# B1ueber2y/DIST-Renderer

Hardware: NVIDIA B200
Metric: rays/sec (fwd+bwd) (higher is better)
Workload: dtype f32 (split-fp16 tensor-core operands, fp32 accumulate)

## Files before the change

### dist-renderer_b200/csrc/common.cuh

```cuda
#pragma once
#include <cuda_runtime.h>
#include <stdint.h>
#include "../../include/dist_b200.h"

namespace dist {

void set_error(const char* fmt, ...);
int num_sms();
void count_launch();

#define DIST_CHECK_CUDA(expr)                                                                   \
  do {                                                                                          \
    cudaError_t _e = (expr);                                                                    \
    if (_e != cudaSuccess) {                                                                    \
      ::dist::set_error("%s failed: %s (%s:%d)", #expr, cudaGetErrorString(_e), __FILE__, __LINE__); \
      return DIST_E_CUDA;                                                                       \
    }                                                                                           \
  } while (0)

#define DIST_REQUIRE(cond, ...)                 \
  do {                                          \
    if (!(cond)) {                              \
      ::dist::set_error(__VA_ARGS__);           \
      return DIST_E_INVALID;                    \
    }                                           \
  } while (0)

__host__ __device__ inline int round_up(int x, int m) { return (x + m - 1) / m * m; }

struct NetDev {
  int n_layers, latent_in, use_tanh;
  int K[DIST_MAX_LAYERS], N[DIST_MAX_LAYERS];
  const float* Wt[DIST_MAX_LAYERS];
  const float* W[DIST_MAX_LAYERS];
  const float* bias[DIST_MAX_LAYERS];
};

int make_netdev(const dist_net_t* net, NetDev* out);

struct MlpArgs {
  const float* points;
  int64_t n_host;
  const int32_t* n_dev;
  float clamp_dist;
  float* sdf;
  float* grad;
  const float* coef;
  const uint8_t* use_clamp;
  float* acc0;
  float* accl;
  int64_t* rows_evaluated;
  int64_t n2_host;
  const int32_t* n2_dev;
  int64_t seg2_offset;
  int screen_seg1;
  float screen_thresh;
  uint8_t* seg_approx;
  unsigned long long* tile_counters;
  uint32_t* mask_buf;
  int64_t mask_cap;
  int64_t mask_base_host;
  const int32_t* mask_base_dev;
  const int32_t* slots;
  const float* sdf_in;
};
int mlp_simt_launch(const NetDev& net, int mode, const MlpArgs& a, cudaStream_t stream);
int mlp_tc_launch(const dist_net_t* net, const NetDev& nd, int mode, const MlpArgs& a, cudaStream_t stream);

int mlp_launch(const dist_net_t* net, const NetDev& nd, int engine, int mode, const MlpArgs& a, cudaStream_t stream);

}
```

### dist-renderer_b200/csrc/march.cu

```cuda
#include <cuda_runtime.h>
#include <math.h>
#include <string.h>
#include "common.cuh"

namespace dist {
namespace {

struct Cam {
  float Kinv[9], M[9], Mn[9];
  const float* R;
  const float* c;
  int W, H, row0, row_step, n_rows, row_group;
  int n_views, Pv;
  float radius;
};

enum { LVL_APPROX = 0x80, LVL_REQUERIED = 0x40 };
enum { VS_LIVE0 = 0, VS_STEPS = 1, VS_MAXENTRY = 2, VS_NONFINITE = 3, VS_STRIDE = 4 };

__device__ __forceinline__ void load_view(const Cam& cam, int v, float (&R)[9], float (&c)[3]) {
#pragma unroll
  for (int i = 0; i < 9; ++i) R[i] = cam.R[9 * v + i];
#pragma unroll
  for (int i = 0; i < 3; ++i) c[i] = cam.c[3 * v + i];
}
__device__ __forceinline__ void load_view_pos(const Cam& cam, int v, float (&c)[3]) {
#pragma unroll
  for (int i = 0; i < 3; ++i) c[i] = cam.c[3 * v + i];
}
__host__ __device__ inline int seg_capacity(int P) { return (P + 1 + 127) / 128 * 128; }

__device__ __forceinline__ void view_atomic_add(int32_t* view_stat, int slot, int v) {
  const unsigned peers = __match_any_sync(0xffffffffu, v);
  if (v >= 0 && (int)(threadIdx.x & 31) == __ffs(peers) - 1) atomicAdd(view_stat + VS_STRIDE * v + slot, __popc(peers));
}
__device__ __forceinline__ void view_atomic_max(int32_t* view_stat, int slot, int v, int value) {
  const unsigned peers = __match_any_sync(0xffffffffu, v);
  if (v >= 0 && (int)(threadIdx.x & 31) == __ffs(peers) - 1) atomicMax(view_stat + VS_STRIDE * v + slot, value);
}

__device__ __forceinline__ int warp_append(int32_t* counter, bool pred) {
  const unsigned m = __ballot_sync(0xffffffffu, pred);
  if (m == 0) return -1;
  const int lane = threadIdx.x & 31;
  const int leader = __ffs(m) - 1;
  int base = 0;
  if (lane == leader) base = atomicAdd(counter, __popc(m));
  base = __shfl_sync(0xffffffffu, base, leader);
  return pred ? base + __popc(m & ((1u << lane) - 1)) : -1;
}

__device__ __forceinline__ void warp_append2(int32_t* counters, bool p1, bool p2, int& idx1, int& idx2) {
  const unsigned m1 = __ballot_sync(0xffffffffu, p1), m2 = __ballot_sync(0xffffffffu, p2);
  idx1 = idx2 = -1;
  if ((m1 | m2) == 0) return;
  const int lane = threadIdx.x & 31;
  const int leader = __ffs(m1 | m2) - 1;
  unsigned long long base = 0;
  if (lane == leader)
    base = atomicAdd(reinterpret_cast<unsigned long long*>(counters),
                     (unsigned long long)__popc(m1) | ((unsigned long long)__popc(m2) << 32));
  base = __shfl_sync(0xffffffffu, base, leader);
  const unsigned below = (1u << lane) - 1;
  if (p1) idx1 = (int)(uint32_t)base + __popc(m1 & below);
  if (p2) idx2 = (int)(uint32_t)(base >> 32) + __popc(m2 & below);
}

__device__ __forceinline__ void coord_ray(const Cam& cam, const float* R, float x, float y, float (&ray)[3]) {
  float hc[3], v[3];
#pragma unroll
  for (int i = 0; i < 3; ++i) hc[i] = fmaf(cam.Kinv[i * 3 + 2], 1.f, fmaf(cam.Kinv[i * 3 + 1], y, cam.Kinv[i * 3] * x));
#pragma unroll
  for (int i = 0; i < 3; ++i) v[i] = fmaf(R[6 + i], hc[2], fmaf(R[3 + i], hc[1], R[i] * hc[0]));
  const float nrm = sqrtf(v[0] * v[0] + v[1] * v[1] + v[2] * v[2]) + 1e-12f;
#pragma unroll
  for (int i = 0; i < 3; ++i) ray[i] = v[i] / nrm;
}
__device__ __forceinline__ int global_row(const Cam& cam, int l) {
  return cam.row0 + (l / cam.row_group) * cam.row_step + (l % cam.row_group);
}
__device__ __forceinline__ void pixel_ray(const Cam& cam, const float* R, int lpv, float (&ray)[3]) {
  coord_ray(cam, R, (float)(lpv % cam.W), (float)global_row(cam, lpv / cam.W), ray);
}

__device__ __forceinline__ void sphere_geom(const float (&c)[3], const float (&ray)[3], float radius, float& dist, bool& hit,
                                            float& entry, float& ex) {
  const float ptq = (c[0] * ray[0] + c[1] * ray[1]) + c[2] * ray[2];
  const float d0 = c[0] - ptq * ray[0], d1 = c[1] - ptq * ray[1], d2 = c[2] - ptq * ray[2];
  dist = sqrtf(d0 * d0 + d1 * d1 + d2 * d2);
  hit = dist <= radius;
  const float value = radius * radius - dist * dist;
  const float chord = (value >= 0.f) ? 2.f * sqrtf(value) : 0.f;
  const float cd = sqrtf((c[0] * c[0] + c[1] * c[1]) + c[2] * c[2]);
  entry = (cd < radius) ? 0.f : sqrtf(cd * cd - dist * dist) - chord / 2.0f;
  ex = entry + chord;
}

__device__ __forceinline__ void topk_insert(const dist_workspace_t& ws, int P, int B, int lp, float sdf, float px, float py,
                                            float pz, float zafter, float zgen, int lvl, int slot = -1) {
  const float asdf = fabsf(sdf);
  int pos = 0;
  float worst = -1.f;
  for (int b = 0; b < B; ++b) {
    const float a = fabsf(ws.top_sdf[(size_t)b * P + lp]);
    if (a >= worst) { worst = a; pos = b; }
  }
  if (!(asdf < worst)) return;
  ws.top_sdf[(size_t)pos * P + lp] = sdf;
  ws.top_zafter[(size_t)pos * P + lp] = zafter;
  ws.top_zgen[(size_t)pos * P + lp] = zgen;
  ws.top_lvl[(size_t)pos * P + lp] = (uint8_t)lvl;
  if (ws.top_slot) ws.top_slot[(size_t)pos * P + lp] = slot;
  ws.top_pt[((size_t)pos * 3 + 0) * P + lp] = px;
  ws.top_pt[((size_t)pos * 3 + 1) * P + lp] = py;
  ws.top_pt[((size_t)pos * 3 + 2) * P + lp] = pz;
}

struct Level {
  int w, h, Pv, P, scale;
  float *ray, *start, *z, *s_sdf, *s_pt, *s_zabs, *s_zgen;
  uint8_t* hit;
  int32_t* list;
  int32_t* count;
  int32_t* s_slot;
};

__device__ __forceinline__ void point_on_ray(const Cam& cam, const float (&c)[3], const float (&ray)[3], float depth,
                                             float (&p)[3]) {
  float q[3];
#pragma unroll
  for (int i = 0; i < 3; ++i) q[i] = ray[i] * depth + c[i];
#pragma unroll
  for (int i = 0; i < 3; ++i) p[i] = fmaf(cam.M[6 + i], q[2], fmaf(cam.M[3 + i], q[1], cam.M[i] * q[0]));
}

__device__ __forceinline__ float clampf(float v, float c) { return fminf(fmaxf(v, -c), c); }

constexpr int BLK_W = 16, BLK_H = 8;
__host__ __device__ inline int setup_threads_per_view(int W, int n_rows) {
  return ((W + BLK_W - 1) / BLK_W) * ((n_rows + BLK_H - 1) / BLK_H) * (BLK_W * BLK_H);
}

__global__ void k_setup(Cam cam, dist_march_t mp, dist_workspace_t ws, float* Zdepth, uint8_t* mask, float* min_sdf,
                        int P, Level L1, Level L2) {
  const int tpv = setup_threads_per_view(cam.W, cam.n_rows);
  const int gi = blockIdx.x * blockDim.x + threadIdx.x;
  const int vv = gi / tpv, r = gi - vv * tpv;
  const int wb = (cam.W + BLK_W - 1) / BLK_W;
  const int blk = r / (BLK_W * BLK_H), inb = r % (BLK_W * BLK_H);
  const int bx = (blk % wb) * BLK_W + inb % BLK_W, by = (blk / wb) * BLK_H + inb / BLK_W;
  const bool in = vv < cam.n_views && bx < cam.W && by < cam.n_rows;
  const int lp = in ? vv * cam.Pv + by * cam.W + bx : 0;
  const bool pyr = mp.marching_type == DIST_MARCH_PYRAMID;
  float R[9], c[3] = {0.f, 0.f, 0.f};
  const int v = in ? lp / cam.Pv : 0, lpv = lp - v * cam.Pv;
  bool live = false;
  float ray[3] = {0.f, 0.f, 1.f}, start = 0.f;
  if (in) {
    load_view(cam, v, R, c);
    pixel_ray(cam, R, lpv, ray);
    float dist, entry, ex;
    bool hit;
    sphere_geom(c, ray, cam.radius, dist, hit, entry, ex);
    start = entry;
    ws.ray[lp] = ray[0]; ws.ray[P + lp] = ray[1]; ws.ray[2 * P + lp] = ray[2];
    ws.exit_[lp] = ex; ws.dist[lp] = dist; ws.z[lp] = 0.f;
    ws.flags[lp] = hit ? 1 : 0;
    ws.nreal[lp] = 0;
    if (ws.sprev) ws.sprev[lp] = 0.f;
    for (int b = 0; b < mp.buffer_size; ++b) {
      ws.top_sdf[(size_t)b * P + lp] = 1.0f;
      ws.top_zafter[(size_t)b * P + lp] = 0.f;
      ws.top_zgen[(size_t)b * P + lp] = nanf("");
      ws.top_lvl[(size_t)b * P + lp] = 0;
      if (ws.top_slot) ws.top_slot[(size_t)b * P + lp] = -1;
#pragma unroll
      for (int k = 0; k < 3; ++k) ws.top_pt[((size_t)b * 3 + k) * P + lp] = 0.f;
    }
    if (pyr) {
      const int x = lpv % cam.W, y = lpv / cam.W;
      const int p1 = v * L1.Pv + (y >> 1) * L1.w + (x >> 1), p2 = v * L2.Pv + (y >> 2) * L2.w + (x >> 2);
      start = L1.start[p1] + (L1.hit[p1] ? L1.z[p1] : 0.f);
      if (hit) {
        for (int lv = 2; lv >= 1; --lv) {
          const Level& L = (lv == 2) ? L2 : L1;
          const int pp = (lv == 2) ? p2 : p1;
          if (!L.hit[pp]) continue;
          const int ns = mp.coarse_steps[2 - lv];
          for (int st = 0; st < ns; ++st)
            topk_insert(ws, P, mp.buffer_size, lp, L.s_sdf[(size_t)st * L.P + pp], L.s_pt[((size_t)st * 3 + 0) * L.P + pp],
                        L.s_pt[((size_t)st * 3 + 1) * L.P + pp], L.s_pt[((size_t)st * 3 + 2) * L.P + pp],
                        L.s_zabs[(size_t)st * L.P + pp] - entry, L.s_zgen[(size_t)st * L.P + pp], lv,
                        L.s_slot[(size_t)st * L.P + pp]);
        }
      }
    }
    ws.entry[lp] = start; ws.entry0[lp] = entry;
    if (!hit) {
      Zdepth[lp] = 1e11f; mask[lp] = 0;
      min_sdf[lp] = dist + mp.threshold - cam.radius;
    }
    live = hit && (mp.marching_type == DIST_MARCH_TRIVIAL || (0.f + start < ex));
  }
  view_atomic_add(ws.view_stat, VS_LIVE0, live ? v : -1);
  const int idx = warp_append(ws.counts + 0, live);
  if (idx >= 0) {
    float p[3];
    point_on_ray(cam, c, ray, start + 0.f, p);
    ws.list_a[idx] = lp;
    ws.pts[(size_t)idx * 3] = p[0]; ws.pts[(size_t)idx * 3 + 1] = p[1]; ws.pts[(size_t)idx * 3 + 2] = p[2];
  }
}

__global__ void k_hit_flags(Cam cam, dist_workspace_t ws, int P) {
  const int lp = blockIdx.x * blockDim.x + threadIdx.x;
  if (lp >= P) return;
  float R[9], c[3], ray[3], dist, entry, ex;
  bool hit;
  const int v = lp / cam.Pv;
  load_view(cam, v, R, c);
  pixel_ray(cam, R, lp - v * cam.Pv, ray);
  sphere_geom(c, ray, cam.radius, dist, hit, entry, ex);
  ws.flags[lp] = hit ? 1 : 0;
}

__global__ void k_pyr_rays(Cam cam, Level L, const uint8_t* fine_hit, int fine_w, int fine_h, int32_t* view_stat) {
  const int i = blockIdx.x * blockDim.x + threadIdx.x;
  if (i >= L.P) return;
  const int v = i / L.Pv, il = i - v * L.Pv;
  const int ix = il % L.w, iy = il / L.w;
  float R[9], c[3], ray[3], dist, entry, ex;
  bool ownhit;
  load_view(cam, v, R, c);
  const float off = ((float)L.scale - 1.f) / 2.f;
  coord_ray(cam, R, (float)L.scale * (float)ix + off, (float)global_row(cam, L.scale * iy) + off, ray);
  sphere_geom(c, ray, cam.radius, dist, ownhit, entry, ex);
  L.ray[i] = ray[0]; L.ray[L.P + i] = ray[1]; L.ray[2 * L.P + i] = ray[2];
  bool pooled = false;
  for (int dy = 0; dy < 2; ++dy)
    for (int dx = 0; dx < 2; ++dx) {
      const int fx = 2 * ix + dx, fy = 2 * iy + dy;
      if (fx < fine_w && fy < fine_h) pooled |= (fine_hit[(size_t)v * fine_w * fine_h + fy * fine_w + fx] & 1) != 0;
    }
  L.hit[i] = pooled ? 1 : 0;
  L.z[i] = 0.f;
  L.start[i] = ownhit ? entry : -1.f;
  if (view_stat && ownhit) atomicMax(view_stat + VS_STRIDE * v + VS_MAXENTRY, __float_as_int(fmaxf(entry, 0.f)));
}

__global__ void k_pyr_global_maxentry(Cam cam, int w2, int h2, int32_t* view_stat) {
  const int i = blockIdx.x * blockDim.x + threadIdx.x;
  const int n = w2 * h2;
  if (i >= n * cam.n_views) return;
  const int v = i / n, il = i - v * n;
  float R[9], c[3], ray[3], dist, entry, ex;
  bool hit;
  load_view(cam, v, R, c);
  coord_ray(cam, R, 4.f * (float)(il % w2) + 1.5f, 4.f * (float)(il / w2) + 1.5f, ray);
  sphere_geom(c, ray, cam.radius, dist, hit, entry, ex);
  if (hit) atomicMax(view_stat + VS_STRIDE * v + VS_MAXENTRY, __float_as_int(fmaxf(entry, 0.f)));
}

__global__ void k_pyr_start(Cam cam, Level L, Level parent, int has_parent, const int32_t* view_stat, float* pts) {
  const int i = blockIdx.x * blockDim.x + threadIdx.x;
  bool on = false;
  float start = 0.f;
  const int v = (i < L.P) ? i / L.Pv : 0;
  if (i < L.P) {
    if (has_parent) {
      const int il = i - v * L.Pv;
      const int ix = il % L.w, iy = il / L.w, pp = v * parent.Pv + (iy >> 1) * parent.w + (ix >> 1);
      start = parent.start[pp] + (parent.hit[pp] ? parent.z[pp] : 0.f);
    } else {
      start = (L.start[i] >= 0.f) ? L.start[i] : __int_as_float(view_stat[VS_STRIDE * v + VS_MAXENTRY]);
    }
    L.start[i] = start;
    on = L.hit[i] != 0;
  }
  const int idx = warp_append(L.count, on);
  if (idx >= 0) {
    float c[3], ray[3] = {L.ray[i], L.ray[L.P + i], L.ray[2 * L.P + i]}, p[3];
    load_view_pos(cam, v, c);
    point_on_ray(cam, c, ray, start + 0.f, p);
    L.list[idx] = i;
    pts[(size_t)idx * 3] = p[0]; pts[(size_t)idx * 3 + 1] = p[1]; pts[(size_t)idx * 3 + 2] = p[2];
  }
}

__global__ void k_pyr_step(Cam cam, dist_march_t mp, Level L, int step, float* pts, const float* sdfbuf, int64_t slot_base,
                           int64_t slot_cap) {
  const int n = *L.count;
  for (int i = blockIdx.x * blockDim.x + threadIdx.x; i < n; i += gridDim.x * blockDim.x) {
    const int id = L.list[i];
    L.s_slot[(size_t)step * L.P + id] = (slot_base >= 0 && slot_base + i < slot_cap) ? (int32_t)(slot_base + i) : -1;
    float c[3];
    load_view_pos(cam, id / L.Pv, c);
    const float sdf = sdfbuf[i];
    const float zc = L.z[id], start = L.start[id];
    const float znew = zc + clampf(sdf, mp.clamp_dist) * mp.ratio;
    L.z[id] = znew;
    L.s_sdf[(size_t)step * L.P + id] = sdf;
#pragma unroll
    for (int k = 0; k < 3; ++k) L.s_pt[((size_t)step * 3 + k) * L.P + id] = pts[(size_t)i * 3 + k];
    L.s_zabs[(size_t)step * L.P + id] = znew + start;
    L.s_zgen[(size_t)step * L.P + id] = start + zc;
    float ray[3] = {L.ray[id], L.ray[L.P + id], L.ray[2 * L.P + id]}, p[3];
    point_on_ray(cam, c, ray, start + znew, p);
    pts[(size_t)i * 3] = p[0]; pts[(size_t)i * 3 + 1] = p[1]; pts[(size_t)i * 3 + 2] = p[2];
  }
}

__global__ void k_append_origin(dist_workspace_t ws, int SEG, int mask_slots_used) {
  ws.pts[(size_t)SEG * 3] = 0.f; ws.pts[(size_t)SEG * 3 + 1] = 0.f; ws.pts[(size_t)SEG * 3 + 2] = 0.f;
  ws.counts[1] = 1;
  if (ws.mask_base) ws.mask_base[0] = mask_slots_used;
}

__global__ void k_march_update(Cam cam, dist_march_t mp, dist_workspace_t ws, int step, int P) {
  const int SEG = seg_capacity(P);
  const int n1 = ws.counts[2 * step];
  const int n2 = (step == 0) ? 0 : ws.counts[2 * step + 1];
  const int n = n1 + n2;
  const bool scr = ws.seg_approx != nullptr;
  const int32_t* cur = (step & 1) ? ws.list_b : ws.list_a;
  int32_t* nxt = (step & 1) ? ws.list_a : ws.list_b;
  const float* pts_cur = ws.pts + (size_t)(step & 1) * (size_t)(2 * SEG) * 3;
  float* pts_nxt = ws.pts + (size_t)((step + 1) & 1) * (size_t)(2 * SEG) * 3;
  if (step == 0 && blockIdx.x == 0 && threadIdx.x == 0) ws.sdf_origin[0] = ws.sdf[SEG];
  const bool mc = scr && ws.mask_buf != nullptr;
  const int mbase = mc ? ws.mask_base[step] : 0;
  if (mc && blockIdx.x == 0 && threadIdx.x == 0)
    ws.mask_base[step + 1] = mbase + (ws.counts[2 * step + 1] + 127) / 128 * 128;
  const int B = mp.buffer_size;
  const float far_thresh = mp.clamp_dist + mp.screen_margin;
  for (int base = blockIdx.x * blockDim.x; base < n; base += gridDim.x * blockDim.x) {
    const int j = base + threadIdx.x;
    bool live = false, approx = false, pred_far = false;
    int lp = 0, v = -1;
    float znew = 0.f, entry = 0.f;
    if (j < n) {
      const int i = (j < n1) ? j : SEG + (j - n1);
      lp = cur[i];
      v = lp / cam.Pv;
      const float sdf = ws.sdf[i];
      const float px = pts_cur[(size_t)i * 3], py = pts_cur[(size_t)i * 3 + 1], pz = pts_cur[(size_t)i * 3 + 2];
      const float zc = ws.z[lp];
      entry = ws.entry[lp];
      znew = zc + clampf(sdf, mp.clamp_dist) * mp.ratio;
      ws.z[lp] = znew;
      ws.nreal[lp] = step + 1;
      if (step == 0 && sdf > mp.threshold) ws.flags[lp] |= 2;
      const float asdf = fabsf(sdf);
      approx = scr && ws.seg_approx[i >> 6] != 0;
      if (scr) {
        const float ext = sdf + (sdf - ws.sprev[lp]);
        pred_far = asdf > mp.screen_tpred ||
                   (step >= 1 && asdf > far_thresh && fabsf(ext) > far_thresh + mp.screen_ext_margin && (ext > 0.f) == (sdf > 0.f));
        ws.sprev[lp] = sdf;
      }
      if (!(asdf <= 1.0f)) atomicOr(ws.view_stat + VS_STRIDE * v + VS_NONFINITE, 1);
      const float zstore = (mp.marching_type == DIST_MARCH_PYRAMID) ? (znew + entry) - ws.entry0[lp] : znew;
      int slot = -1;
      if (mc && i >= SEG && (int64_t)mbase + (i - SEG) < ws.mask_cap) slot = mbase + (i - SEG);
      topk_insert(ws, P, B, lp, sdf, px, py, pz, zstore, entry + zc, approx ? LVL_APPROX : 0, slot);
      if (step + 1 < mp.march_step) {
        if (mp.marching_type == DIST_MARCH_TRIVIAL) live = true;
        else live = (znew + entry < ws.exit_[lp]) && (asdf >= mp.threshold);
      }
    }
    view_atomic_max(ws.view_stat, VS_STEPS, v, step + 1);
    const bool to1 = live && (!scr || pred_far), to2 = live && !to1;
    float p[3] = {0.f, 0.f, 0.f};
    if (live) {
      float ray[3] = {ws.ray[lp], ws.ray[P + lp], ws.ray[2 * P + lp]}, c[3];
      load_view_pos(cam, v, c);
      point_on_ray(cam, c, ray, entry + znew, p);
    }
    int idx, idx2;
    warp_append2(ws.counts + 2 * (step + 1), to1, to2, idx, idx2);
    if (idx2 >= 0) idx = SEG + idx2;
    if (idx >= 0) {
      nxt[idx] = lp;
      pts_nxt[(size_t)idx * 3] = p[0]; pts_nxt[(size_t)idx * 3 + 1] = p[1]; pts_nxt[(size_t)idx * 3 + 2] = p[2];
    }
  }
}

__global__ void k_requery_gen(dist_march_t mp, dist_workspace_t ws, int P) {
  const int lp = blockIdx.x * blockDim.x + threadIdx.x;
  const bool on = lp < P && (ws.flags[lp] & 1);
  const int B = mp.buffer_size;
  const float E = 0.5f * mp.screen_margin;
  float U = 3.0e38f;
  if (on)
    for (int b = 0; b < B; ++b)
      U = fminf(U, fabsf(ws.top_sdf[(size_t)b * P + lp]) + ((ws.top_lvl[(size_t)b * P + lp] & LVL_APPROX) ? E : 0.f));
  for (int b = 0; b < B; ++b) {
    const bool cand = on && (ws.top_lvl[(size_t)b * P + lp] & LVL_APPROX) && (fabsf(ws.top_sdf[(size_t)b * P + lp]) - E <= U);
    const int idx = warp_append(ws.rq_cnt, cand);
    if (idx >= 0) {
      ws.rq_idx[idx] = lp * DIST_MAX_BUFFER + b;
#pragma unroll
      for (int k = 0; k < 3; ++k) ws.rq_pts[(size_t)idx * 3 + k] = ws.top_pt[((size_t)b * 3 + k) * P + lp];
    }
  }
}

__global__ void k_requery_apply(dist_workspace_t ws, int P, int base_index) {
  const int n = *ws.rq_cnt;
  const bool mc = ws.mask_buf != nullptr && ws.top_slot != nullptr;
  const int mbase = mc ? ws.mask_base[base_index] : 0;
  for (int i = blockIdx.x * blockDim.x + threadIdx.x; i < n; i += gridDim.x * blockDim.x) {
    const int lp = ws.rq_idx[i] / DIST_MAX_BUFFER, b = ws.rq_idx[i] % DIST_MAX_BUFFER;
    ws.top_sdf[(size_t)b * P + lp] = ws.rq_sdf[i];
    if (mc) ws.top_slot[(size_t)b * P + lp] = ((int64_t)mbase + i < ws.mask_cap) ? mbase + i : -1;
    ws.top_lvl[(size_t)b * P + lp] = (uint8_t)((ws.top_lvl[(size_t)b * P + lp] & ~LVL_APPROX) | LVL_REQUERIED);
  }
}

__global__ void k_finalize(dist_march_t mp, dist_workspace_t ws, float* Zdepth, uint8_t* mask, float* min_sdf, int P, int Pv) {
  const int lp = blockIdx.x * blockDim.x + threadIdx.x;
  if (lp >= P || !(ws.flags[lp] & 1)) return;
  const int B = mp.buffer_size;
  const int S = ws.view_stat[VS_STRIDE * (lp / Pv) + VS_STEPS];
  int nreal = ws.nreal[lp];
  const float so = ws.sdf_origin[0];
  const float zfin = ws.z[lp];
  if (S < B && nreal == S && nreal > 0) {
    const float zkey = (mp.marching_type == DIST_MARCH_PYRAMID) ? (zfin + ws.entry[lp]) - ws.entry0[lp] : zfin;
    int j = -1;
    for (int b = 0; b < B; ++b)
      if (ws.top_zafter[(size_t)b * P + lp] == zkey && (ws.top_lvl[(size_t)b * P + lp] & 3) == 0 &&
          ws.top_sdf[(size_t)b * P + lp] != 1.0f) j = b;
    if (j >= 0) {
      const float r_sdf = ws.top_sdf[(size_t)j * P + lp], r_za = ws.top_zafter[(size_t)j * P + lp],
                  r_zg = ws.top_zgen[(size_t)j * P + lp];
      const float r_p[3] = {ws.top_pt[((size_t)j * 3 + 0) * P + lp], ws.top_pt[((size_t)j * 3 + 1) * P + lp],
                            ws.top_pt[((size_t)j * 3 + 2) * P + lp]};
      const int r_lvl = ws.top_lvl[(size_t)j * P + lp];
      const int r_slot = ws.top_slot ? ws.top_slot[(size_t)j * P + lp] : -1;
      for (int i = 0; i < B - S; ++i) topk_insert(ws, P, B, lp, r_sdf, r_p[0], r_p[1], r_p[2], r_za, r_zg, r_lvl, r_slot);
    }
    nreal = B;
    ws.nreal[lp] = B;
  }
  {
    float key[DIST_MAX_BUFFER];
    int ord[DIST_MAX_BUFFER];
#pragma unroll
    for (int b = 0; b < DIST_MAX_BUFFER; ++b) {
      key[b] = (b < B) ? fabsf(ws.top_sdf[(size_t)b * P + lp]) : 0.f;
      ord[b] = b;
    }
    bool moved = false;
#pragma unroll
    for (int a = 1; a < DIST_MAX_BUFFER; ++a) {
      if (a < B) {
        bool go = true;
#pragma unroll
        for (int b = a; b > 0; --b) {
          go = go && (key[b] < key[b - 1]);
          if (go) {
            const float tk = key[b]; key[b] = key[b - 1]; key[b - 1] = tk;
            const int to = ord[b]; ord[b] = ord[b - 1]; ord[b - 1] = to;
            moved = true;
          }
        }
      }
    }
    if (moved) {
      auto permute_f = [&](float* base, size_t stride) {
        float v[DIST_MAX_BUFFER];
#pragma unroll
        for (int b = 0; b < DIST_MAX_BUFFER; ++b) v[b] = (b < B) ? base[(size_t)b * stride + lp] : 0.f;
#pragma unroll
        for (int d = 0; d < DIST_MAX_BUFFER; ++d) {
          if (d < B && ord[d] != d) {
            float o = 0.f;
#pragma unroll
            for (int sidx = 0; sidx < DIST_MAX_BUFFER; ++sidx) o = (ord[d] == sidx) ? v[sidx] : o;
            base[(size_t)d * stride + lp] = o;
          }
        }
      };
      permute_f(ws.top_sdf, (size_t)P);
      permute_f(ws.top_zafter, (size_t)P);
      permute_f(ws.top_zgen, (size_t)P);
      for (int k = 0; k < 3; ++k) permute_f(ws.top_pt + (size_t)k * P, (size_t)3 * P);
      {
        int v[DIST_MAX_BUFFER];
#pragma unroll
        for (int b = 0; b < DIST_MAX_BUFFER; ++b) v[b] = (b < B) ? (int)ws.top_lvl[(size_t)b * P + lp] : 0;
#pragma unroll
        for (int d = 0; d < DIST_MAX_BUFFER; ++d) {
          if (d < B && ord[d] != d) {
            int o = 0;
#pragma unroll
            for (int sidx = 0; sidx < DIST_MAX_BUFFER; ++sidx) o = (ord[d] == sidx) ? v[sidx] : o;
            ws.top_lvl[(size_t)d * P + lp] = (uint8_t)o;
          }
        }
      }
      if (ws.top_slot) {
        int v[DIST_MAX_BUFFER];
#pragma unroll
        for (int b = 0; b < DIST_MAX_BUFFER; ++b) v[b] = (b < B) ? ws.top_slot[(size_t)b * P + lp] : -1;
#pragma unroll
        for (int d = 0; d < DIST_MAX_BUFFER; ++d) {
          if (d < B && ord[d] != d) {
            int o = -1;
#pragma unroll
            for (int sidx = 0; sidx < DIST_MAX_BUFFER; ++sidx) o = (ord[d] == sidx) ? v[sidx] : o;
            ws.top_slot[(size_t)d * P + lp] = o;
          }
        }
      }
    }
  }
  const float s0 = ws.top_sdf[lp];
  const float entry = ws.entry[lp];
  const bool real0 = (s0 != 1.0f);
  const bool first_ok = (nreal == 0) || (ws.flags[lp] & 2);
  const bool valid = (zfin + entry < ws.exit_[lp]) && (fabsf(s0) <= mp.threshold) &&
                     (!mp.first_query_check || first_ok);
  min_sdf[lp] = real0 ? s0 : so;
  float zz = ws.top_zafter[lp] + (1.f - mp.ratio) * clampf(s0, mp.clamp_dist);
  const int vw = lp / Pv;
  if ((mp.replay_grad_rounding >> 31) & 1 || (vw < 31 && ((mp.replay_grad_rounding >> vw) & 1))) {
    for (int b = 0; b < B; ++b) {
      const float sb = ws.top_sdf[(size_t)b * P + lp];
      const float s = clampf((sb != 1.0f) ? sb : so, mp.clamp_dist);
      const float a = s * mp.ratio;
      zz = zz - a;
      zz = zz + a;
    }
  }
  Zdepth[lp] = ws.entry0[lp] + zz;
  mask[lp] = valid ? 1 : 0;
}

__global__ void k_normal_gen(Cam cam, const float* Zdepth, const uint8_t* mask, int32_t* idx_out, float* pts,
                             int32_t* count, int P) {
  const int lp = blockIdx.x * blockDim.x + threadIdx.x;
  const bool on = lp < P && mask[lp] != 0;
  const int idx = warp_append(count, on);
  if (idx >= 0) {
    float R[9], c[3], ray[3], p[3];
    const int v = lp / cam.Pv;
    load_view(cam, v, R, c);
    pixel_ray(cam, R, lp - v * cam.Pv, ray);
    point_on_ray(cam, c, ray, Zdepth[lp], p);
    idx_out[idx] = lp;
    pts[(size_t)idx * 3] = p[0]; pts[(size_t)idx * 3 + 1] = p[1]; pts[(size_t)idx * 3 + 2] = p[2];
  }
}

__global__ void k_normal_finish(Cam cam, const int32_t* idx_in, const float* grad, const int32_t* count, int normalize,
                                float* Znormal, int P) {
  const int n = *count;
  for (int i = blockIdx.x * blockDim.x + threadIdx.x; i < n; i += gridDim.x * blockDim.x) {
    const int lp = idx_in[i];
    float g[3] = {grad[(size_t)i * 3], grad[(size_t)i * 3 + 1], grad[(size_t)i * 3 + 2]};
    if (normalize) {
      const float nrm = sqrtf(g[0] * g[0] + g[1] * g[1] + g[2] * g[2]) + 1e-12f;
      g[0] = g[0] / nrm; g[1] = g[1] / nrm; g[2] = g[2] / nrm;
    }
#pragma unroll
    for (int k = 0; k < 3; ++k)
      Znormal[(size_t)k * P + lp] = fmaf(cam.Mn[k * 3 + 2], g[2], fmaf(cam.Mn[k * 3 + 1], g[1], cam.Mn[k * 3] * g[0]));
  }
}

__global__ void k_bwd_gen(dist_march_t mp, dist_workspace_t ws, const float* gZ, const float* gM, int32_t* row_pix,
                          float* pts, float* coef, int32_t* count, int P, int use_masks) {
  const int lp = blockIdx.x * blockDim.x + threadIdx.x;
  const bool hit = lp < P && (ws.flags[lp] & 1);
  const int B = mp.buffer_size;
  const float so = ws.sdf_origin[0];
  const float gz = (hit && gZ) ? gZ[lp] : 0.f;
  const float gm = (hit && gM) ? gM[lp] : 0.f;
  for (int b = 0; b < B; ++b) {
    float cf = 0.f, s = 0.f;
    int slot = -1;
    if (hit) {
      const float sb = ws.top_sdf[(size_t)b * P + lp];
      s = (sb != 1.0f) ? sb : so;
      const bool cm = (s >= -mp.clamp_dist) && (s <= mp.clamp_dist);
      cf = cm ? mp.ratio * gz : 0.f;
      if (b == 0) cf += gm;
      if (use_masks && sb != 1.0f) slot = ws.top_slot[(size_t)b * P + lp];
    }
    const int idx = warp_append(count, cf != 0.f && slot < 0);
    if (idx >= 0) {
      row_pix[idx] = lp * DIST_MAX_BUFFER + b;
      coef[idx] = cf;
#pragma unroll
      for (int k = 0; k < 3; ++k) pts[(size_t)idx * 3 + k] = ws.top_pt[((size_t)b * 3 + k) * P + lp];
    }
    if (use_masks) {
      const int im = warp_append(ws.bm_cnt, cf != 0.f && slot >= 0);
      if (im >= 0) { ws.bm_row[im] = lp * DIST_MAX_BUFFER + b; ws.bm_slot[im] = slot; ws.bm_sdf[im] = s; ws.bm_coef[im] = cf; }
    }
  }
}

__global__ void k_bwd_scatter(Cam cam, dist_workspace_t ws, const int32_t* row_pix, const float* dpts,
                              const int32_t* count, float* d_cam, float* d_ray, float* d_ray_coarse, int w1, int P1v, int w2,
                              int P2v, int P, int cam_levels) {
  const int n = *count;
  const size_t P1 = (size_t)cam.n_views * P1v, P2 = (size_t)cam.n_views * P2v;
  float acc[3] = {0.f, 0.f, 0.f};
  int acc_v = -1;
  for (int i = blockIdx.x * blockDim.x + threadIdx.x; i < n; i += gridDim.x * blockDim.x) {
    const int lp = row_pix[i] / DIST_MAX_BUFFER, b = row_pix[i] % DIST_MAX_BUFFER;
    const float zg = ws.top_zgen[(size_t)b * P + lp];
    if (zg != zg) continue;
    const int lvl = ws.top_lvl[(size_t)b * P + lp] & 3;
    if (!((cam_levels >> (lvl ? 1 : 0)) & 1)) continue;
    const int v = lp / cam.Pv, lpv = lp - v * cam.Pv;
    if (v != acc_v) {
      if (acc_v >= 0)
        for (int k = 0; k < 3; ++k)
          if (acc[k] != 0.f) atomicAdd(d_cam + 3 * acc_v + k, acc[k]);
      acc[0] = acc[1] = acc[2] = 0.f;
      acc_v = v;
    }
    const float d[3] = {dpts[(size_t)i * 3], dpts[(size_t)i * 3 + 1], dpts[(size_t)i * 3 + 2]};
#pragma unroll
    for (int k = 0; k < 3; ++k) {
      const float g = fmaf(cam.M[k * 3 + 2], d[2], fmaf(cam.M[k * 3 + 1], d[1], cam.M[k * 3] * d[0]));
      acc[k] += g;
      if (lvl == 0) atomicAdd(d_ray + (size_t)k * P + lp, g * zg);
      else if (d_ray_coarse) {
        const int x = lpv % cam.W, y = lpv / cam.W;
        if (lvl == 1) atomicAdd(d_ray_coarse + (size_t)k * P1 + (size_t)v * P1v + (y >> 1) * w1 + (x >> 1), g * zg);
        else atomicAdd(d_ray_coarse + 3 * P1 + (size_t)k * P2 + (size_t)v * P2v + (y >> 2) * w2 + (x >> 2), g * zg);
      }
    }
  }
  const unsigned same = __match_any_sync(0xffffffffu, acc_v);
  const bool uniform = (same == 0xffffffffu);
#pragma unroll
  for (int k = 0; k < 3; ++k) {
    float t = acc[k];
    if (uniform) {
      for (int o = 16; o > 0; o >>= 1) t += __shfl_xor_sync(0xffffffffu, t, o);
      if ((threadIdx.x & 31) == 0 && acc_v >= 0 && t != 0.f) atomicAdd(d_cam + 3 * acc_v + k, t);
    } else if (acc_v >= 0 && t != 0.f) {
      atomicAdd(d_cam + 3 * acc_v + k, t);
    }
  }
}

int make_cam(const dist_camera_t* cam, Cam* out) {
  DIST_REQUIRE(cam && cam->R && cam->cam_pos, "camera: null pointer");
  DIST_REQUIRE(cam->width > 0 && cam->n_rows > 0 && cam->row_step > 0, "camera: bad image/tile description");
  const int n_views = cam->n_views > 0 ? cam->n_views : 1;
  DIST_REQUIRE((int64_t)cam->width * cam->n_rows * n_views < (int64_t)(1u << 31) / DIST_MAX_BUFFER, "camera: tile too large");
  for (int i = 0; i < 9; ++i) { out->Kinv[i] = cam->Kinv[i]; out->M[i] = cam->M[i]; out->Mn[i] = cam->Mn[i]; }
  out->R = cam->R; out->c = cam->cam_pos;
  out->W = cam->width; out->H = cam->height; out->row0 = cam->row0; out->row_step = cam->row_step;
  out->n_rows = cam->n_rows; out->radius = cam->radius;
  out->row_group = cam->row_group > 0 ? cam->row_group : 1;
  DIST_REQUIRE(cam->row0 >= 0 && cam->row0 + ((cam->n_rows - 1) / out->row_group) * cam->row_step + (cam->n_rows - 1) % out->row_group < cam->height,
               "camera: row band outside the image");
  out->n_views = n_views; out->Pv = cam->width * cam->n_rows;
  return DIST_OK;
}

}

static void carve_levels(const Cam& cam, const dist_workspace_t* ws, Level* L1, Level* L2) {
  Level* Ls[2] = {L1, L2};
  int w = cam.W, h = cam.n_rows;
  float* f = ws->pyr_f;
  int32_t* li = ws->pyr_i;
  uint8_t* bb = ws->pyr_b;
  const int w1 = (w + 1) / 2, h1 = (h + 1) / 2, w2 = (w1 + 1) / 2, h2 = (h1 + 1) / 2;
  const int dims[2][2] = {{w1, h1}, {w2, h2}};
  int32_t* slots = li + ((size_t)w1 * h1 + (size_t)w2 * h2) * cam.n_views;
  int32_t* counts = li + 4 * ((size_t)w1 * h1 + (size_t)w2 * h2) * cam.n_views;
  for (int i = 0; i < 2; ++i) {
    Level& L = *Ls[i];
    L.w = dims[i][0]; L.h = dims[i][1]; L.Pv = L.w * L.h; L.P = L.Pv * cam.n_views; L.scale = (i == 0) ? 2 : 4;
    L.ray = f; f += 3 * (size_t)L.P;
    L.start = f; f += L.P;
    L.z = f; f += L.P;
    L.s_sdf = f; f += 3 * (size_t)L.P;
    L.s_pt = f; f += 9 * (size_t)L.P;
    L.s_zabs = f; f += 3 * (size_t)L.P;
    L.s_zgen = f; f += 3 * (size_t)L.P;
    L.hit = bb; bb += L.P;
    L.list = li; li += L.P;
    L.s_slot = slots; slots += 3 * (size_t)L.P;
    L.count = counts + i;
  }
}

int render_depth_fwd(const dist_net_t* net, int engine, const dist_camera_t* camh, const dist_march_t* mp_in,
                     const dist_workspace_t* ws, float* Zdepth, uint8_t* mask, float* min_sdf, int64_t* rows_eval,
                     cudaStream_t st) {
  Cam cam;
  int rc = make_cam(camh, &cam);
  if (rc) return rc;
  NetDev nd;
  rc = make_netdev(net, &nd);
  if (rc) return rc;
  dist_march_t mpv = *mp_in;
  dist_march_t* mp = &mpv;
  DIST_REQUIRE(mp->buffer_size >= 1 && mp->buffer_size <= DIST_MAX_BUFFER, "buffer_size must be in [1,%d]", DIST_MAX_BUFFER);
  DIST_REQUIRE(mp->march_step >= 1, "march_step must be >= 1");
  DIST_REQUIRE(mp->marching_type >= DIST_MARCH_TRIVIAL && mp->marching_type <= DIST_MARCH_PYRAMID, "bad marching_type");
  DIST_REQUIRE(ws->entry0 && ws->top_lvl && ws->view_stat, "workspace: entry0 / top_lvl / view_stat missing");
  const bool pyr = mp->marching_type == DIST_MARCH_PYRAMID;
  const int P = cam.Pv * cam.n_views;
  DIST_CHECK_CUDA(cudaMemsetAsync(ws->view_stat, 0, sizeof(int32_t) * VS_STRIDE * cam.n_views, st));
  const int S_total = mp->march_step;
  const int tb = 256, gb = (P + tb - 1) / tb;
  const bool scr = mp->screen != 0 && engine == DIST_ENGINE_TC;
  const int SEG = seg_capacity(P);
  dist_workspace_t wsv = *ws;
  if (scr) {
    DIST_REQUIRE(ws->seg_approx && ws->sprev && ws->rq_idx && ws->rq_pts && ws->rq_sdf && ws->rq_cnt,
                 "workspace: two-tier precision buffers missing");
    DIST_REQUIRE(mp->screen_margin > 0.f && mp->screen_tpred >= mp->clamp_dist && mp->screen_ext_margin >= 0.f,
                 "two-tier precision: bad margin / prediction thresholds");
    DIST_CHECK_CUDA(cudaMemsetAsync(ws->rq_cnt, 0, sizeof(int32_t), st));
  } else {
    wsv.seg_approx = nullptr;
  }
  const bool mc = scr && ws->mask_buf != nullptr;
  if (mc) {
    DIST_REQUIRE(ws->mask_base && ws->top_slot && ws->mask_cap > 0 && ws->mask_cap < (int64_t)1 << 31, "workspace: mask cache buffers missing");
    DIST_CHECK_CUDA(cudaMemsetAsync(ws->mask_base, 0, sizeof(int32_t) * (S_total + 3), st));
  } else {
    wsv.mask_buf = nullptr; wsv.top_slot = nullptr;
  }
  ws = &wsv;
  Level L1, L2;
  memset(&L1, 0, sizeof(L1)); memset(&L2, 0, sizeof(L2));
  int64_t coarse_slots = 0;
  if (pyr) {
    DIST_REQUIRE(ws->pyr_f && ws->pyr_i && ws->pyr_b, "workspace: pyramid buffers missing");
    const bool full_image = cam.row0 == 0 && cam.row_step == cam.row_group && cam.n_rows == cam.H;
    DIST_REQUIRE(full_image || cam.row_group % 4 == 0,
                 "pyramid marching on a row band needs bands made of 4-row groups (row_group % 4 == 0) so that the 1/2- and "
                 "1/4-resolution levels stay band-local");
    DIST_REQUIRE(mp->coarse_steps[0] >= 1 && mp->coarse_steps[0] <= 3 && mp->coarse_steps[1] >= 1 && mp->coarse_steps[1] <= 3 &&
                     mp->coarse_steps[0] + mp->coarse_steps[1] < S_total, "pyramid marching: coarse step counts must be in [1,3]");
    carve_levels(cam, ws, &L1, &L2);
    mp->march_step = S_total - mp->coarse_steps[0] - mp->coarse_steps[1];
    mp->first_query_check = 0;
    DIST_CHECK_CUDA(cudaMemsetAsync(L1.count, 0, sizeof(int32_t) * 8, st));
    k_hit_flags<<<gb, tb, 0, st>>>(cam, *ws, P); count_launch();
    k_pyr_rays<<<(L1.P + tb - 1) / tb, tb, 0, st>>>(cam, L1, ws->flags, cam.W, cam.n_rows, nullptr); count_launch();
    k_pyr_rays<<<(L2.P + tb - 1) / tb, tb, 0, st>>>(cam, L2, L1.hit, L1.w, L1.h, full_image ? ws->view_stat : nullptr); count_launch();
    if (!full_image) {
      const int w2g = ((cam.W + 1) / 2 + 1) / 2, h2g = ((cam.H + 1) / 2 + 1) / 2;
      k_pyr_global_maxentry<<<(w2g * h2g * cam.n_views + tb - 1) / tb, tb, 0, st>>>(cam, w2g, h2g, ws->view_stat); count_launch();
    }
    for (int lv = 2; lv >= 1; --lv) {
      Level& L = (lv == 2) ? L2 : L1;
      k_pyr_start<<<(L.P + tb - 1) / tb, tb, 0, st>>>(cam, L, L2, lv == 1 ? 1 : 0, ws->view_stat, ws->pts); count_launch();
      const int ns = mp->coarse_steps[2 - lv];
      for (int s = 0; s < ns; ++s) {
        MlpArgs a{};
        a.points = ws->pts; a.n_host = L.P; a.n_dev = L.count; a.clamp_dist = 0.f; a.sdf = ws->sdf; a.rows_evaluated = rows_eval;
        a.tile_counters = ws->tile_counters;
        const int64_t slot_base = mc ? coarse_slots : -1;
        if (mc) { a.mask_buf = ws->mask_buf; a.mask_cap = ws->mask_cap; a.mask_base_host = slot_base; coarse_slots += (L.P + 127) / 128 * 128; }
        rc = mlp_launch(net, nd, engine, 0, a, st);
        if (rc) return rc;
        k_pyr_step<<<min((L.P + tb - 1) / tb, 4 * num_sms()), tb, 0, st>>>(cam, *mp, L, s, ws->pts, ws->sdf, slot_base,
                                                                           mc ? ws->mask_cap : 0); count_launch();
      }
    }
  }
  const int S = mp->march_step;
  DIST_CHECK_CUDA(cudaMemsetAsync(ws->counts, 0, sizeof(int32_t) * 2 * (S_total + 2), st));
  k_setup<<<(cam.n_views * setup_threads_per_view(cam.W, cam.n_rows) + tb - 1) / tb, tb, 0, st>>>(cam, *mp, *ws, Zdepth, mask, min_sdf, P,
                                                                                                L1, L2); count_launch();
  k_append_origin<<<1, 1, 0, st>>>(*ws, SEG, (int)coarse_slots); count_launch();
  DIST_CHECK_CUDA(cudaGetLastError());
  const int gu = min(gb, 4 * num_sms());
  for (int s = 0; s < S; ++s) {
    MlpArgs a{};
    a.points = ws->pts + (size_t)(s & 1) * (size_t)(2 * SEG) * 3;
    a.n_host = P; a.n_dev = ws->counts + 2 * s;
    a.n2_host = P + 1; a.n2_dev = ws->counts + 2 * s + 1; a.seg2_offset = SEG;
    a.clamp_dist = 0.f; a.sdf = ws->sdf; a.rows_evaluated = rows_eval;
    a.tile_counters = ws->tile_counters;
    if (scr) { a.screen_seg1 = 1; a.screen_thresh = mp->clamp_dist + mp->screen_margin; a.seg_approx = ws->seg_approx; }
    if (mc) { a.mask_buf = ws->mask_buf; a.mask_cap = ws->mask_cap; a.mask_base_dev = ws->mask_base + s; }
    rc = mlp_launch(net, nd, engine, 0, a, st);
    if (rc) return rc;
    k_march_update<<<gu, tb, 0, st>>>(cam, *mp, *ws, s, P); count_launch();
  }
  if (scr) {
    k_requery_gen<<<gb, tb, 0, st>>>(*mp, *ws, P); count_launch();
    MlpArgs a{};
    a.points = ws->rq_pts; a.n_host = (int64_t)P * mp->buffer_size; a.n_dev = ws->rq_cnt; a.clamp_dist = 0.f; a.sdf = ws->rq_sdf;
    a.tile_counters = ws->tile_counters;
    if (mc) { a.mask_buf = ws->mask_buf; a.mask_cap = ws->mask_cap; a.mask_base_dev = ws->mask_base + S; }
    rc = mlp_launch(net, nd, engine, 0, a, st);
    if (rc) return rc;
    k_requery_apply<<<gu, tb, 0, st>>>(*ws, P, S); count_launch();
  }
  k_finalize<<<gb, tb, 0, st>>>(*mp, *ws, Zdepth, mask, min_sdf, P, cam.Pv); count_launch();
  DIST_CHECK_CUDA(cudaGetLastError());
  return DIST_OK;
}

int render_normal_fwd(const dist_net_t* net, int engine, const dist_camera_t* camh, const float* Zdepth,
                      const uint8_t* mask, float clamp_dist, int normalize, float* Znormal, int32_t* s_idx,
                      float* s_pts, float* s_grad, int32_t* s_count, int64_t* rows_eval, cudaStream_t st) {
  Cam cam;
  int rc = make_cam(camh, &cam);
  if (rc) return rc;
  NetDev nd;
  rc = make_netdev(net, &nd);
  if (rc) return rc;
  const int P = cam.Pv * cam.n_views;
  DIST_CHECK_CUDA(cudaMemsetAsync(s_count, 0, sizeof(int32_t), st));
  DIST_CHECK_CUDA(cudaMemsetAsync(Znormal, 0, sizeof(float) * 3 * (size_t)P, st));
  const int tb = 256, gb = (P + tb - 1) / tb;
  k_normal_gen<<<gb, tb, 0, st>>>(cam, Zdepth, mask, s_idx, s_pts, s_count, P); count_launch();
  MlpArgs a{};
  a.points = s_pts; a.n_host = P; a.n_dev = s_count; a.clamp_dist = clamp_dist; a.grad = s_grad;
  a.rows_evaluated = rows_eval;
  rc = mlp_launch(net, nd, engine, 1, a, st);
  if (rc) return rc;
  k_normal_finish<<<min(gb, 4 * num_sms()), tb, 0, st>>>(cam, s_idx, s_grad, s_count, normalize, Znormal, P); count_launch();
  DIST_CHECK_CUDA(cudaGetLastError());
  return DIST_OK;
}

int render_depth_bwd(const dist_net_t* net, int engine, const dist_camera_t* camh, const dist_march_t* mp,
                     const dist_workspace_t* ws, const float* gZ, const float* gM, float* acc0, float* accl,
                     float* d_cam, float* d_ray, float* d_ray_coarse, int32_t* s_row_pix, float* s_pts, float* s_coef, uint8_t* s_clamp,
                     float* s_dpts, int32_t* s_count, int64_t* rows_eval, cudaStream_t st) {
  (void)s_clamp;
  Cam cam;
  int rc = make_cam(camh, &cam);
  if (rc) return rc;
  NetDev nd;
  rc = make_netdev(net, &nd);
  if (rc) return rc;
  const int P = cam.Pv * cam.n_views;
  DIST_CHECK_CUDA(cudaMemsetAsync(s_count, 0, sizeof(int32_t), st));
  const int tb = 256, gb = (P + tb - 1) / tb;
  const bool mc = engine == DIST_ENGINE_TC && ws->mask_buf && ws->top_slot && ws->bm_row && ws->bm_slot && ws->bm_sdf && ws->bm_coef &&
                  ws->bm_dpts && ws->bm_cnt;
  if (mc) DIST_CHECK_CUDA(cudaMemsetAsync(ws->bm_cnt, 0, sizeof(int32_t), st));
  k_bwd_gen<<<gb, tb, 0, st>>>(*mp, *ws, gZ, gM, s_row_pix, s_pts, s_coef, s_count, P, mc ? 1 : 0); count_launch();
  MlpArgs a{};
  a.points = s_pts; a.n_host = (int64_t)P * mp->buffer_size; a.n_dev = s_count; a.clamp_dist = 0.f;
  a.grad = s_dpts; a.coef = s_coef; a.acc0 = acc0; a.accl = accl; a.rows_evaluated = rows_eval;
  rc = mlp_launch(net, nd, engine, 2, a, st);
  if (rc) return rc;
  if (mc) {
    MlpArgs b{};
    b.n_host = (int64_t)P * mp->buffer_size; b.n_dev = ws->bm_cnt; b.clamp_dist = 0.f;
    b.grad = ws->bm_dpts; b.coef = ws->bm_coef; b.acc0 = acc0; b.accl = accl;
    b.rows_evaluated = rows_eval ? rows_eval + 1 : nullptr;
    b.mask_buf = ws->mask_buf; b.mask_cap = ws->mask_cap; b.slots = ws->bm_slot; b.sdf_in = ws->bm_sdf;
    rc = mlp_launch(net, nd, engine, 3, b, st);
    if (rc) return rc;
  }
  if (d_cam && d_ray) {
    const int w1 = (cam.W + 1) / 2, h1 = (cam.n_rows + 1) / 2, w2 = (w1 + 1) / 2, h2 = (h1 + 1) / 2;
    const int gs = min((int)(((int64_t)P * mp->buffer_size + tb - 1) / tb), 4 * num_sms());
    const int lv = mp->cam_grad_levels ? mp->cam_grad_levels : 3;
    k_bwd_scatter<<<gs, tb, 0, st>>>(cam, *ws, s_row_pix, s_dpts, s_count, d_cam, d_ray, d_ray_coarse, w1, w1 * h1, w2, w2 * h2, P, lv);
    count_launch();
    if (mc) {
      k_bwd_scatter<<<gs, tb, 0, st>>>(cam, *ws, ws->bm_row, ws->bm_dpts, ws->bm_cnt, d_cam, d_ray, d_ray_coarse, w1, w1 * h1, w2,
                                       w2 * h2, P, lv);
      count_launch();
    }
  }
  DIST_CHECK_CUDA(cudaGetLastError());
  return DIST_OK;
}

}
```

### dist-renderer_b200/csrc/mlp_tc.cu

```cuda
#include <cuda.h>
#include <cuda_fp16.h>
#include <cuda_runtime.h>
#include <stdio.h>
#include <stdlib.h>
#include <string.h>
#include "common.cuh"

namespace dist {
namespace {

#ifdef DIST_TC_TIMELINE
#define TL_BEGIN() const long long tl_c0 = clock64()
#define TL_TILE (c1 > 0 ? 2 : 1)
#define TL_END(slot_) do { if (io.dbg_out && cluster_id == 0 && i == TL_TILE && lane == 0) io.dbg_out[256 + 2 * m + (slot_)] += clock64() - tl_c0; } while (0)
#define TL_MARK(idx_) do { if (io.dbg_out && cluster_id == 0 && i == TL_TILE && lane == 0) io.dbg_out[idx_] = clock64(); } while (0)
#else
#define TL_BEGIN() do {} while (0)
#define TL_END(slot_) do {} while (0)
#define TL_MARK(idx_) do {} while (0)
#endif

constexpr int NST = 6;
constexpr int STAGE_BYTES = 16384;
constexpr int OFF_AHI = 0, OFF_ALO = 65536, OFF_W = 131072;
constexpr int OFF_BAR = OFF_W + NST * STAGE_BYTES;
constexpr int OFF_HDR = OFF_BAR + 448;
constexpr int OFF_PART = OFF_BAR + 512;
constexpr int OFF_ROWD = OFF_PART + 2048;
constexpr int OFF_FAIL = OFF_ROWD + 256;
constexpr int FAIL_WORDS = 32;
constexpr int SMEM_BYTES = OFF_FAIL + 16 + 4 * FAIL_WORDS;
constexpr int NTHREADS = 640;
constexpr int MAX_PROG = 2 * 10;

struct LayerTC {
  int kc32;
  int nh;
  int stage_base;
  int N;
  int app_xyz;
  float inv_scale;
  const float* bias;
};

struct TcParams {
  int n_mma;
  int n_prog;
  int acc_l_prog;
  int accl_N;
  LayerTC L[MAX_PROG];
  const float* w0;
  const float* bias0;
  int N0, N0p4;
  const float* wlast;
  const float* blast;
  int K_last;
  int use_tanh;
  float sA, sD;
  int first_append;
  int dbg;
  int stage_rows;
};

struct TcIO {
  const float* points; int64_t n_host; const int32_t* n_dev; float clamp_dist;
  int64_t n2_host; const int32_t* n2_dev; int64_t seg2_offset;
  float* sdf; float* grad; const float* coef; const uint8_t* use_clamp; float* acc0; float* accl;
  int64_t* rows_evaluated;
  long long* dbg_out;
  int screen_seg1;
  float screen_thresh;
  uint8_t* seg_approx;
  unsigned long long* tile_counters;
  uint32_t* mask_buf;
  int64_t mask_cap;
  int64_t mask_base_host;
  const int32_t* mask_base_dev;
  const int32_t* slots;
  const float* sdf_in;
};

__device__ __forceinline__ uint32_t smem_u32(const void* p) { return (uint32_t)__cvta_generic_to_shared(p); }
__device__ __forceinline__ uint32_t cluster_ctarank() { uint32_t r; asm volatile("mov.u32 %0, %%cluster_ctarank;" : "=r"(r)); return r; }
__device__ __forceinline__ void cluster_sync_all() {
  asm volatile("barrier.cluster.arrive.release.aligned;\n" ::: "memory");
  asm volatile("barrier.cluster.wait.acquire.aligned;\n" ::: "memory");
}
__device__ __forceinline__ void mbar_init(uint32_t bar, uint32_t count) { asm volatile("mbarrier.init.shared::cta.b64 [%0], %1;" ::"r"(bar), "r"(count)); }
__device__ __forceinline__ void mbar_expect_tx(uint32_t bar, uint32_t bytes) {
  asm volatile("mbarrier.arrive.expect_tx.shared::cta.b64 _, [%0], %1;" ::"r"(bar), "r"(bytes) : "memory");
}
__device__ __forceinline__ void mbar_wait(uint32_t bar, uint32_t parity) {
  asm volatile(
      "{\n.reg .pred p;\nWAIT_%=:\n"
      "mbarrier.try_wait.parity.shared::cta.b64 p, [%0], %1;\n"
      "@p bra DONE_%=;\nbra WAIT_%=;\nDONE_%=:\n}\n" ::"r"(bar), "r"(parity) : "memory");
}
__device__ __forceinline__ void mbar_wait_cluster(uint32_t bar, uint32_t parity) {
  asm volatile(
      "{\n.reg .pred p;\nWAIT_%=:\n"
      "mbarrier.try_wait.parity.shared::cta.b64 p, [%0], %1;\n"
      "@p bra DONE_%=;\nbra WAIT_%=;\nDONE_%=:\n}\n" ::"r"(bar), "r"(parity) : "memory");
}
__device__ __forceinline__ void mbar_arrive_cluster(uint32_t bar_local, uint32_t target_rank) {
  uint32_t remote;
  asm volatile("mapa.shared::cluster.u32 %0, %1, %2;" : "=r"(remote) : "r"(bar_local), "r"(target_rank));
  asm volatile("mbarrier.arrive.shared::cluster.b64 _, [%0];" ::"r"(remote) : "memory");
}
__device__ __forceinline__ uint32_t ld_dsmem_u32(uint32_t local_addr, uint32_t rank) {
  uint32_t remote, v;
  asm volatile("mapa.shared::cluster.u32 %0, %1, %2;" : "=r"(remote) : "r"(local_addr), "r"(rank));
  asm volatile("ld.shared::cluster.u32 %0, [%1];" : "=r"(v) : "r"(remote) : "memory");
  return v;
}
__device__ __forceinline__ uint64_t make_desc(uint32_t saddr, uint32_t lbo, uint32_t sbo) {
  uint64_t d = 0;
  d |= (uint64_t)((saddr & 0x3FFFF) >> 4);
  d |= (uint64_t)(lbo >> 4) << 16;
  d |= (uint64_t)(sbo >> 4) << 32;
  d |= (uint64_t)1 << 46;
  return d;
}
__device__ __forceinline__ void mma_f16_2cta(uint32_t tmem_d, uint64_t da, uint64_t db, uint32_t idesc, uint32_t acc) {
  asm volatile(
      "{\n.reg .pred p;\nsetp.ne.b32 p, %4, 0;\n"
      "tcgen05.mma.cta_group::2.kind::f16 [%0], %1, %2, %3, p;\n}\n" ::"r"(tmem_d), "l"(da), "l"(db), "r"(idesc), "r"(acc)
      : "memory");
}
__device__ __forceinline__ void commit_mc(uint32_t bar) {
  asm volatile("tcgen05.commit.cta_group::2.mbarrier::arrive::one.shared::cluster.multicast::cluster.b64 [%0], %1;" ::"r"(bar),
               "h"((uint16_t)3)
               : "memory");
}
__device__ __forceinline__ bool elect_one() {
  uint32_t pred;
  asm volatile("{\n.reg .pred p;\nelect.sync _|p, 0xffffffff;\nselp.u32 %0, 1, 0, p;\n}\n" : "=r"(pred));
  return pred != 0;
}
__device__ __forceinline__ void tc_fence_before() { asm volatile("tcgen05.fence::before_thread_sync;" ::: "memory"); }
__device__ __forceinline__ void tc_fence_after() { asm volatile("tcgen05.fence::after_thread_sync;" ::: "memory"); }
__device__ __forceinline__ void epi_bar_sync() { asm volatile("bar.sync 1, 512;" ::: "memory"); }

__device__ __forceinline__ void tmem_ld32(uint32_t taddr, float (&v)[32]) {
  uint32_t r[32];
  asm volatile(
      "tcgen05.ld.sync.aligned.32x32b.x32.b32 {%0,%1,%2,%3,%4,%5,%6,%7,%8,%9,%10,%11,%12,%13,%14,%15,%16,%17,%18,%19,%20,%21,%22,"
      "%23,%24,%25,%26,%27,%28,%29,%30,%31}, [%32];"
      : "=r"(r[0]), "=r"(r[1]), "=r"(r[2]), "=r"(r[3]), "=r"(r[4]), "=r"(r[5]), "=r"(r[6]), "=r"(r[7]), "=r"(r[8]), "=r"(r[9]),
        "=r"(r[10]), "=r"(r[11]), "=r"(r[12]), "=r"(r[13]), "=r"(r[14]), "=r"(r[15]), "=r"(r[16]), "=r"(r[17]), "=r"(r[18]),
        "=r"(r[19]), "=r"(r[20]), "=r"(r[21]), "=r"(r[22]), "=r"(r[23]), "=r"(r[24]), "=r"(r[25]), "=r"(r[26]), "=r"(r[27]),
        "=r"(r[28]), "=r"(r[29]), "=r"(r[30]), "=r"(r[31])
      : "r"(taddr));
  asm volatile("tcgen05.wait::ld.sync.aligned;" ::: "memory");
#pragma unroll
  for (int i = 0; i < 32; ++i) v[i] = __uint_as_float(r[i]);
}

__device__ __forceinline__ void store_group(uint8_t* smem, int feat0, int row, const float* x) {
  __half2 h[4], l[4];
#pragma unroll
  for (int i = 0; i < 4; ++i) {
    h[i] = __floats2half2_rn(x[2 * i], x[2 * i + 1]);
    const float2 hf = __half22float2(h[i]);
    l[i] = __floats2half2_rn(x[2 * i] - hf.x, x[2 * i + 1] - hf.y);
  }
  const int off = (feat0 >> 3) * 1024 + row * 16;
  *reinterpret_cast<uint4*>(smem + OFF_AHI + off) = *reinterpret_cast<uint4*>(h);
  *reinterpret_cast<uint4*>(smem + OFF_ALO + off) = *reinterpret_cast<uint4*>(l);
}

__device__ __forceinline__ void store_group_hi(uint8_t* smem, int region, int feat0, int row, const float* x) {
  __half2 h[4];
#pragma unroll
  for (int i = 0; i < 4; ++i) h[i] = __floats2half2_rn(x[2 * i], x[2 * i + 1]);
  *reinterpret_cast<uint4*>(smem + region + (feat0 >> 3) * 1024 + row * 16) = *reinterpret_cast<uint4*>(h);
}

template <int MODE>
__global__ void __cluster_dims__(2, 1, 1) __launch_bounds__(NTHREADS, 1)
mlp_tc_kernel(const __grid_constant__ CUtensorMap tmap, const __grid_constant__ CUtensorMap tmap_hi, const TcParams P, const TcIO io) {
  extern __shared__ __align__(1024) uint8_t smem[];
  volatile int64_t* hdr = reinterpret_cast<volatile int64_t*>(smem + OFF_HDR);
  if (threadIdx.x == 0) {
    const int64_t v0 = io.n_dev ? (int64_t)*io.n_dev : io.n_host;
    const int64_t v1 = io.n2_dev ? (int64_t)*io.n2_dev : io.n2_host;
    const int64_t v2 = (MODE == 0 && io.mask_buf) ? (io.mask_base_dev ? (int64_t)*io.mask_base_dev : io.mask_base_host) : -1;
    hdr[0] = v0; hdr[1] = v1; hdr[2] = v2;
  }
  __syncthreads();
  const int64_t n1 = hdr[0], n2 = hdr[1];
  const int64_t n = n1 + n2;
  if (n <= 0) return;
  const uint32_t rank = cluster_ctarank();
  const int tid = threadIdx.x, warp = tid >> 5, lane = tid & 31;
  const int cluster_id = blockIdx.x >> 1, n_clusters = gridDim.x >> 1;
  const int64_t tiles1 = (n1 + 127) / 128, n_tiles = tiles1 + (n2 + 127) / 128;
  if ((blockIdx.x >> 1) >= n_tiles) return;
  auto row0_of = [&](int64_t t) -> int64_t { return (t < tiles1) ? t * 128 : io.seg2_offset + (t - tiles1) * 128; };
  auto lim_of = [&](int64_t t) -> int64_t { return (t < tiles1) ? n1 : io.seg2_offset + n2; };
  if (blockIdx.x == 0 && tid == 0 && io.rows_evaluated)
    atomicAdd(reinterpret_cast<unsigned long long*>(io.rows_evaluated), (unsigned long long)n);
  const int64_t mask_base = hdr[2];

  long long dbg_c0 = 0, dbg_t0 = 0;
  if (io.dbg_out && blockIdx.x == 0 && tid == 0) { dbg_c0 = clock64(); asm volatile("mov.u64 %0, %%globaltimer;" : "=l"(dbg_t0)); }
  const uint32_t sbase = smem_u32(smem);
  const uint32_t bar0 = sbase + OFF_BAR;
  auto W_FULL = [&](int s) { return bar0 + 8 * s; };
  auto W_EMPTY = [&](int s) { return bar0 + 8 * (NST + s); };
  auto A_FULL = [&](int c) { return bar0 + 8 * (2 * NST + c); };
  auto A_FREE = [&](int c) { return bar0 + 8 * (2 * NST + 16 + c); };
  auto D_FULL = [&](int b, int h) { return bar0 + 8 * (2 * NST + 32 + 2 * b + h); };
  const uint32_t FIN = bar0 + 8 * (2 * NST + 36);
  uint32_t* tmem_slot = reinterpret_cast<uint32_t*>(smem + OFF_BAR + 8 * (2 * NST + 37));
  const int n_prog = P.n_prog;
  const int m0 = (MODE == 3) ? P.n_mma : 0;

  const int cnt = (cluster_id < n_tiles) ? (int)((n_tiles - cluster_id + n_clusters - 1) / n_clusters) : 0;
  const bool screening = (MODE == 0) && io.screen_seg1 != 0 && cnt <= 32 * FAIL_WORDS;
  volatile uint32_t* near_flag = reinterpret_cast<volatile uint32_t*>(smem + OFF_FAIL);
  volatile uint32_t* fail_words = reinterpret_cast<volatile uint32_t*>(smem + OFF_FAIL + 16);
  const uint32_t fail_addr = sbase + OFF_FAIL + 16;
  auto tile_of = [&](int i) -> int64_t { return cluster_id + (int64_t)i * n_clusters; };
  const int c1 = (screening && cluster_id < tiles1) ? (int)((tiles1 - cluster_id + n_clusters - 1) / n_clusters) : 0;
  auto next_tile = [&](int phase, int i) -> int {
    if (phase == 0) {
      const int j = (i < 0) ? 0 : ((i < c1) ? min(i + 2, c1) : i + 1);
      return (j < cnt) ? j : -1;
    }
    int j = i + 1;
    while (j < cnt) {
      const uint32_t w = (fail_words[j >> 5] | ld_dsmem_u32(fail_addr + 4 * (j >> 5), rank ^ 1u)) >> (j & 31);
      if (w) { j += __ffs(w) - 1; return (j < cnt) ? j : -1; }
      j = (j | 31) + 1;
    }
    return -1;
  };

  if (tid == 0) {
    for (int s = 0; s < NST; ++s) { mbar_init(W_FULL(s), 1); mbar_init(W_EMPTY(s), 1); }
    for (int c = 0; c < 16; ++c) mbar_init(A_FULL(c), 4);
    for (int c = 0; c < 16; ++c) mbar_init(A_FREE(c), 1);
    for (int b = 0; b < 2; ++b) { mbar_init(D_FULL(b, 0), 1); mbar_init(D_FULL(b, 1), 1); }
    mbar_init(FIN, 32);
    near_flag[0] = 0u; near_flag[1] = 0u;
    for (int w = 0; w < FAIL_WORDS; ++w) fail_words[w] = 0u;
    asm volatile("fence.mbarrier_init.release.cluster;" ::: "memory");
  }
  if (warp == 2) {
    asm volatile("tcgen05.alloc.cta_group::2.sync.aligned.shared::cta.b32 [%0], %1;" ::"r"(smem_u32(tmem_slot)), "r"(512) : "memory");
    asm volatile("tcgen05.relinquish_alloc_permit.cta_group::2.sync.aligned;" ::: "memory");
  }
  tc_fence_before();
  __syncthreads();
  cluster_sync_all();
  tc_fence_after();
  const uint32_t tmem = *tmem_slot;

  if (warp == 0) {
    {
      uint32_t p_slot = 0, p_phase = 0;
      const uint32_t bar_leader_mask = 0xFEFFFFFFu;
      for (int phase = 0; phase < 2; ++phase) {
        for (int i = next_tile(phase, -1); i >= 0; i = next_tile(phase, i)) {
          const bool exact = !(phase == 0 && i < c1);
          for (int m = m0; m < n_prog; ++m) {
            const int kc32 = P.L[m].kc32, sb = P.L[m].stage_base;
            const int nslot = exact ? kc32 * P.L[m].nh : (kc32 / 2) * P.L[m].nh;
            for (int s = 0; s < nslot; ++s) {
              const uint32_t slot = p_slot, ph = p_phase;
              if (++p_slot == NST) { p_slot = 0; p_phase ^= 1; }
              mbar_wait(W_EMPTY(slot), ph ^ 1);
              if (elect_one()) {
                if (rank == 0) mbar_expect_tx(W_FULL(slot), 2 * STAGE_BYTES);
                const uint32_t dst = sbase + OFF_W + slot * STAGE_BYTES;
                const uint32_t bar = W_FULL(slot) & bar_leader_mask;
                if (exact) {
                  const int row = ((sb + s) * 2 + (int)rank) * P.stage_rows;
                  asm volatile(
                      "cp.async.bulk.tensor.2d.cta_group::2.shared::cluster.global.mbarrier::complete_tx::bytes [%0], [%1, {%3, %4}], [%2];" ::
                          "r"(dst), "l"(&tmap), "r"(bar), "r"(0), "r"(row)
                      : "memory");
                } else {
#pragma unroll
                  for (int c = 0; c < 2; ++c) {
                    const int row = ((sb + 2 * s + c) * 2 + (int)rank) * P.stage_rows;
                    asm volatile(
                        "cp.async.bulk.tensor.2d.cta_group::2.shared::cluster.global.mbarrier::complete_tx::bytes [%0], [%1, {%3, %4}], [%2];" ::
                            "r"(dst + c * (STAGE_BYTES / 2)), "l"(&tmap_hi), "r"(bar), "r"(0), "r"(row)
                        : "memory");
                  }
                }
              }
              __syncwarp();
            }
          }
        }
        if (phase == 0) {
          if (!screening) break;
          cluster_sync_all();
        }
      }
    }
  } else if (warp == 1) {
    if (rank == 0) {
      const uint32_t idesc = (1u << 4) | ((256u >> 3) << 17) | ((128u >> 4) << 24);
      const uint64_t a_hi0 = make_desc(sbase + OFF_AHI, 1024, 128);
      const uint64_t a_lo0 = make_desc(sbase + OFF_ALO, 1024, 128);
      const uint64_t b_0 = make_desc(sbase + OFF_W, 2048, 128);
      uint32_t G = 0, a_phase = 0, fin_phase = 0, w_slot = 0, w_phase = 0;
      uint32_t d_first = 1;
      bool prev_pair = false;
      for (int phase = 0; phase < 2; ++phase) {
      for (int i = next_tile(phase, -1); i >= 0; i = next_tile(phase, i)) {
        const int64_t t = tile_of(i);
        const bool exact = !(phase == 0 && i < c1);
        const bool has_b = !exact && (i + 1 < c1);
        (void)t;
        for (int m = m0; m < n_prog; ++m, ++G) {
          const int kc32 = P.L[m].kc32, nh = P.L[m].nh;
          const uint32_t buf = exact ? (G & 1) : 0u;
          if (!d_first && m == m0 + ((!exact || prev_pair) ? 0 : 1)) { mbar_wait_cluster(FIN, fin_phase); fin_phase ^= 1; }
          for (int h = 0; h < nh; ++h) {
            const uint32_t d_addr = tmem + buf * 256 + h * 128;
            const bool last_pass = (h == nh - 1);
            if (!exact) {
              for (int kc = 0; kc < kc32; kc += 4) {
                const int nsl = (kc + 2 < kc32) ? 2 : 1;
                if (h == 0) {
                  TL_BEGIN();
                  for (int c = 0; c < 2 * nsl; ++c) mbar_wait_cluster(A_FULL(kc + c), (a_phase >> (kc + c)) & 1);
                  if (kc == 0) TL_MARK(8 + m * 4 + 0);
                  if (kc == 0)
                    for (int c = 2 * nsl; c < min(8, kc32); ++c) mbar_wait_cluster(A_FULL(c), (a_phase >> c) & 1);
                  a_phase ^= (nsl == 2 ? 15u : 3u) << kc;
                  TL_END(0);
                }
                const uint32_t slot0 = w_slot, ph0 = w_phase;
                uint32_t slot1 = slot0, ph1 = ph0;
                if (++w_slot == NST) { w_slot = 0; w_phase ^= 1; }
                if (nsl == 2) {
                  slot1 = w_slot; ph1 = w_phase;
                  if (++w_slot == NST) { w_slot = 0; w_phase ^= 1; }
                }
                {
                  TL_BEGIN();
                  mbar_wait(W_FULL(slot0), ph0);
                  if (nsl == 2) mbar_wait(W_FULL(slot1), ph1);
                  TL_END(1);
                }
                tc_fence_after();
                if (elect_one()) {
                  for (int u = 0; u < nsl; ++u) {
                    const uint32_t slot = u ? slot1 : slot0;
                    for (int ts = 0; ts < (has_b ? 2 : 1); ++ts) {
                      const uint64_t a_base = ts ? a_lo0 : a_hi0;
                      const uint32_t d_ts = d_addr + ts * 256;
#pragma unroll
                      for (int c = 0; c < 2; ++c) {
#pragma unroll
                        for (int ks = 0; ks < 2; ++ks) {
                          const int kk = kc + 2 * u + c;
                          const uint64_t a_off = (uint64_t)((kk * 4 + ks * 2) * 64);
                          const uint64_t b_off = (uint64_t)(slot * (STAGE_BYTES / 16) + c * 512 + ks * 256);
                          mma_f16_2cta(d_ts, a_base + a_off, b_0 + b_off, idesc, (kk | ks) ? 1u : 0u);
                        }
                      }
                    }
                    commit_mc(W_EMPTY(slot));
                    if (last_pass) { commit_mc(A_FREE(kc + 2 * u)); commit_mc(A_FREE(kc + 2 * u + 1)); }
                  }
                  if (kc + 4 >= kc32) commit_mc(D_FULL(buf, h));
                }
                __syncwarp();
                if (kc + 4 >= kc32 && last_pass) TL_MARK(8 + m * 4 + 1);
              }
            } else
            for (int kc = 0; kc < kc32; kc += 2) {
              if (h == 0) {
                TL_BEGIN();
                mbar_wait_cluster(A_FULL(kc), (a_phase >> kc) & 1);
                mbar_wait_cluster(A_FULL(kc + 1), (a_phase >> (kc + 1)) & 1);
                a_phase ^= (3u << kc);
                TL_END(0);
#ifdef DIST_TC_TIMELINE
                if (io.dbg_out && cluster_id == 0 && t == cluster_id + n_clusters && lane == 0 && kc == 0) io.dbg_out[8 + m * 4 + 0] = clock64();
#endif
              }
              const uint32_t slot0 = w_slot, ph0 = w_phase;
              uint32_t slot1 = slot0 + 1, ph1 = ph0;
              if (slot1 == NST) { slot1 = 0; ph1 ^= 1; }
              w_slot = slot1 + 1; w_phase = ph1;
              if (w_slot == NST) { w_slot = 0; w_phase ^= 1; }
              {
                TL_BEGIN();
                mbar_wait(W_FULL(slot0), ph0);
                mbar_wait(W_FULL(slot1), ph1);
                TL_END(1);
              }
              tc_fence_after();
              if (elect_one()) {
#pragma unroll
                for (int u = 0; u < 2; ++u) {
                  const uint32_t slot = u ? slot1 : slot0;
#pragma unroll
                  for (int ks = 0; ks < 2; ++ks) {
                    const uint64_t a_off = (uint64_t)(((kc + u) * 4 + ks * 2) * 64);
                    const uint64_t b_off = (uint64_t)(slot * (STAGE_BYTES / 16) + ks * 256);
                    mma_f16_2cta(d_addr, a_hi0 + a_off, b_0 + b_off, idesc, ((kc + u) | ks) ? 1u : 0u);
                    mma_f16_2cta(d_addr, a_lo0 + a_off, b_0 + b_off, idesc, 1u);
                    mma_f16_2cta(d_addr, a_hi0 + a_off, b_0 + b_off + 512, idesc, 1u);
                  }
                  commit_mc(W_EMPTY(slot));
                  if (last_pass) commit_mc(A_FREE(kc + u));
                }
                if (kc + 2 >= kc32) commit_mc(D_FULL(buf, h));
              }
              __syncwarp();
#ifdef DIST_TC_TIMELINE
              if (io.dbg_out && cluster_id == 0 && t == cluster_id + n_clusters && lane == 0 && kc + 2 >= kc32 && last_pass) io.dbg_out[8 + m * 4 + 1] = clock64();
              if (io.dbg_out && cluster_id == 0 && t == cluster_id && lane == 0 && kc + 2 >= kc32 && last_pass && m == n_prog - 1) io.dbg_out[200] = clock64();
#endif
            }
          }
        }
        d_first = 0;
        prev_pair = !exact;
      }
        if (phase == 0) {
          if (!screening) break;
          cluster_sync_all();
        }
      }
    } else if (screening) {
      cluster_sync_all();
    }
  } else if (warp < 4) {
    if (screening) cluster_sync_all();
  } else {
    const int ew = warp - 4;
    const int qq = warp & 3;
    const int q = qq >> 1;
    const int ch = ew >> 2;
    const int row = 32 * (qq & 1) + lane;
    const uint32_t lane_base = (uint32_t)(32 * qq) << 16;
    const float sA = P.sA, sD = P.sD;
    const int n_mma = P.n_mma;
    float* part = reinterpret_cast<float*>(smem + OFF_PART);
    float* rowd = reinterpret_cast<float*>(smem + OFF_ROWD);
    const int pslot = 4 * q + ch;
    uint32_t G = 0, d_phase = 0, free_phase = 0;
    float px = 0.f, py = 0.f, pz = 0.f;
    uint32_t mk[DIST_MAX_LAYERS][2];
    float acc0r[2] = {0.f, 0.f}, acclr[2] = {0.f, 0.f};

    auto rec_slot = [&](int64_t t) -> int64_t {
      if (MODE != 0 || mask_base < 0) return -1;
      const int64_t r = row0_of(t) + rank * 64 + row;
      if (r >= lim_of(t)) return -1;
      int64_t idx;
      if (io.screen_seg1) { if (t < tiles1) return -1; idx = r - io.seg2_offset; }
      else { if (n2 > 0) return -1; idx = r; }
      const int64_t sl = mask_base + idx;
      return (sl < io.mask_cap) ? sl : -1;
    };
    const bool rec_on = (MODE == 0) && mask_base >= 0;
    auto load_point = [&](int64_t t) {
      const int64_t gr = row0_of(t) + rank * 64 + row;
      if (gr < lim_of(t)) { px = io.points[gr * 3]; py = io.points[gr * 3 + 1]; pz = io.points[gr * 3 + 2]; }
      else { px = py = pz = 0.f; }
    };
    auto signal_block = [&](int kc) {
      asm volatile("fence.proxy.async.shared::cta;" ::: "memory");
      __syncwarp();
      if (lane == 0) mbar_arrive_cluster(A_FULL(kc), 0);
    };
    auto layer0 = [&](int64_t slot, int guard_kc32) {
      const int kblocks = P.L[0].kc32;
      const int nh0 = (P.N0 + 255) >> 8;
      for (int h = 0; h < nh0; ++h) {
        const int kb = 8 * h + 4 * q + ch;
        if (kb >= kblocks) continue;
        const int f0 = 32 * kb;
        uint32_t m0 = 0;
        if (kb < guard_kc32) mbar_wait(A_FREE(kb), (free_phase >> kb) & 1);
#pragma unroll
        for (int g = 0; g < 4; ++g) {
          float x[8];
#pragma unroll
          for (int e = 0; e < 8; ++e) {
            const int f = f0 + 8 * g + e;
            float v = 0.f;
            if (f < P.N0) {
              v = fmaf(__ldg(P.w0 + 2 * P.N0p4 + f), pz, fmaf(__ldg(P.w0 + P.N0p4 + f), py, __ldg(P.w0 + f) * px)) + __ldg(P.bias0 + f);
              if (v > 0.f) m0 |= 1u << (8 * g + e); else v = 0.f;
            } else if (P.first_append && f < P.N0 + 3) {
              v = (f == P.N0) ? px : ((f == P.N0 + 1) ? py : pz);
            }
            x[e] = v * sA;
          }
          store_group(smem, f0 + 8 * g, row, x);
        }
        if (MODE != 0) mk[0][h] = m0;
        if (MODE == 0 && slot >= 0) io.mask_buf[(size_t)kb * io.mask_cap + slot] = m0;
        signal_block(kb);
      }
    };
    auto colsum32 = [&](float (&v)[32]) -> float {
#pragma unroll
      for (int o = 16; o >= 1; o >>= 1) {
        const bool up = (lane & o) != 0;
#pragma unroll
        for (int j = 0; j < o; ++j) {
          const float mine = up ? v[j + o] : v[j];
          const float send = up ? v[j] : v[j + o];
          v[j] = mine + __shfl_xor_sync(0xffffffffu, send, o);
        }
      }
      return v[0];
    };
    auto row_sum8 = [&]() -> float {
      const float* pr = part + row * 8;
      return ((pr[0] + pr[1]) + (pr[2] + pr[3])) + ((pr[4] + pr[5]) + (pr[6] + pr[7]));
    };

    unsigned int n_tiles_1pass = 0, n_tiles_3pass = 0;

    float qx = 0.f, qy = 0.f, qz = 0.f;
    auto load_points_pair = [&](int i) {
      load_point(tile_of(i));
      const int64_t tb = tile_of(i + 1);
      const int64_t grb = row0_of(tb) + rank * 64 + row;
      if (i + 1 < c1 && grb < n1) { qx = io.points[grb * 3]; qy = io.points[grb * 3 + 1]; qz = io.points[grb * 3 + 2]; }
      else { qx = qy = qz = 0.f; }
    };
    auto layer0_pair = [&](int guard_kc32) {
      const int kblocks = P.L[0].kc32;
      const int nh0 = (P.N0 + 255) >> 8;
      for (int h = 0; h < nh0; ++h) {
        const int kb = 8 * h + 4 * q + ch;
        if (kb >= kblocks) continue;
        const int f0 = 32 * kb;
        if (kb < guard_kc32) mbar_wait(A_FREE(kb), (free_phase >> kb) & 1);
#pragma unroll
        for (int g = 0; g < 4; ++g) {
          float xa[8], xb[8];
#pragma unroll
          for (int e = 0; e < 8; ++e) {
            const int f = f0 + 8 * g + e;
            float va = 0.f, vb = 0.f;
            if (f < P.N0) {
              const float wx = __ldg(P.w0 + f), wy = __ldg(P.w0 + P.N0p4 + f), wz = __ldg(P.w0 + 2 * P.N0p4 + f), b = __ldg(P.bias0 + f);
              va = fmaxf(fmaf(wz, pz, fmaf(wy, py, wx * px)) + b, 0.f);
              vb = fmaxf(fmaf(wz, qz, fmaf(wy, qy, wx * qx)) + b, 0.f);
            } else if (P.first_append && f < P.N0 + 3) {
              va = (f == P.N0) ? px : ((f == P.N0 + 1) ? py : pz);
              vb = (f == P.N0) ? qx : ((f == P.N0 + 1) ? qy : qz);
            }
            xa[e] = va * sA; xb[e] = vb * sA;
          }
          store_group_hi(smem, OFF_AHI, f0 + 8 * g, row, xa);
          store_group_hi(smem, OFF_ALO, f0 + 8 * g, row, xb);
        }
        signal_block(kb);
      }
    };
    float seed_scale = 0.f;
    auto seed = [&](int64_t t) {
      const int64_t r = row0_of(t) + rank * 64 + row;
      const bool ok = r < lim_of(t);
      int64_t sl = -1;
      float o = 0.f, cf = 0.f;
      if (ok) { sl = io.slots[r]; o = io.sdf_in[r]; cf = io.coef ? io.coef[r] : 1.f; }
      float d = 1.f - o * o;
      if (P.use_tanh) { const float t1 = atanhf(o); d *= (1.f - t1 * t1); }
      bool uc = io.clamp_dist > 0.f;
      if (io.use_clamp) uc = ok ? (io.use_clamp[r] != 0) : false;
      if (uc && !(o >= -io.clamp_dist && o <= io.clamp_dist)) d = 0.f;
      seed_scale = (ok && sl >= 0) ? d * cf : 0.f;
      for (int l = 0; l <= n_mma; ++l)
#pragma unroll
        for (int h = 0; h < 2; ++h)
          mk[l][h] = (ok && sl >= 0) ? io.mask_buf[((size_t)l * 16 + (8 * h + 4 * q + ch)) * io.mask_cap + sl] : 0u;
      const int LNl = P.L[n_mma - 1].N, kblocks = P.L[n_mma].kc32;
      for (int h = 0; h < 2; ++h) {
        const int kb = 8 * h + 4 * q + ch;
        if (kb >= kblocks) continue;
        const int f0 = 32 * kb;
        const uint32_t mb = mk[n_mma][h];
#pragma unroll
        for (int g = 0; g < 4; ++g) {
          float x[8];
#pragma unroll
          for (int e = 0; e < 8; ++e) {
            const int f = f0 + 8 * g + e;
            x[e] = (f < LNl && ((mb >> (8 * g + e)) & 1u)) ? __ldg(P.wlast + f) * sD : 0.f;
          }
          store_group(smem, f0 + 8 * g, row, x);
        }
        signal_block(kb);
      }
    };
    auto prefetch_points = [&](int phase, int inext) {
      if (inext < 0 || MODE == 3) return;
      if (phase == 0 && inext < c1) load_points_pair(inext); else load_point(tile_of(inext));
    };
    auto start_layer0 = [&](int phase, int inext, int guard_kc32) {
      if (inext < 0) return;
      if (MODE == 3) { seed(tile_of(inext)); return; }
      if (phase == 0 && inext < c1) layer0_pair(guard_kc32); else layer0(rec_slot(tile_of(inext)), guard_kc32);
    };
    auto run_pair = [&](int i, int inext, bool has_b) {
      const int64_t ta = tile_of(i), tb = tile_of(i + 1);
      const int64_t gra = row0_of(ta) + rank * 64 + row, grb = row0_of(tb) + rank * 64 + row;
      const bool oka = gra < n1, okb = has_b && grb < n1;
      float dota = 0.f, dotb = 0.f;
      for (int m = 0; m < n_mma; ++m, ++G) {
        const bool last = (m == n_mma - 1);
        const int LN = P.L[m].N, Lnh = P.L[m].nh, Lapp = P.L[m].app_xyz;
        const float cscale = P.L[m].inv_scale;
        const float* Lbias = P.L[m].bias;
        const int kc32_cur = P.L[m].kc32;
        const int kblocks_next = last ? 0 : P.L[m + 1].kc32;
        auto wait_h = [&](int h) {
          mbar_wait(D_FULL(0, h), (d_phase >> h) & 1);
          d_phase ^= (1u << h);
          tc_fence_after();
        };
        if (last) prefetch_points(0, inext);
        for (int h = 0; h < Lnh; ++h) {
          const int kb = 8 * h + 4 * q + ch;
          const int fb = 32 * kb;
          const bool need_store = !last && kb < kblocks_next;
          const bool process = last ? (fb < LN) : need_store;
          if (last && h == Lnh - 1) start_layer0(0, inext, kc32_cur);
          wait_h(h);
          if (!process) continue;
          const bool interior = (fb + 32 <= LN);
          if (h == 0 && rank == 0 && warp == 4) TL_MARK(8 + m * 4 + 2);
          if (need_store && kb < kc32_cur) mbar_wait(A_FREE(kb), (free_phase >> kb) & 1);
          for (int ts = 0; ts < (has_b ? 2 : 1); ++ts) {
            float v[32];
            tmem_ld32(tmem + lane_base + ts * 256 + h * 128 + 32 * ch, v);
            if (interior) {
#pragma unroll
              for (int j4 = 0; j4 < 8; ++j4) {
                const float4 b4 = __ldg(reinterpret_cast<const float4*>(Lbias + fb) + j4);
                v[4 * j4] = fmaxf(fmaf(v[4 * j4], cscale, b4.x), 0.f);
                v[4 * j4 + 1] = fmaxf(fmaf(v[4 * j4 + 1], cscale, b4.y), 0.f);
                v[4 * j4 + 2] = fmaxf(fmaf(v[4 * j4 + 2], cscale, b4.z), 0.f);
                v[4 * j4 + 3] = fmaxf(fmaf(v[4 * j4 + 3], cscale, b4.w), 0.f);
              }
            } else {
              const float ax = ts ? qx : px, ay = ts ? qy : py, az = ts ? qz : pz;
#pragma unroll
              for (int j = 0; j < 32; ++j) {
                const int f = fb + j;
                float a = 0.f;
                if (f < LN) a = fmaxf(fmaf(v[j], cscale, __ldg(Lbias + f)), 0.f);
                else if (Lapp && f < LN + 3) a = ((f == LN) ? ax : ((f == LN + 1) ? ay : az)) * sA;
                v[j] = a;
              }
            }
            if (last) {
              float d = 0.f;
#pragma unroll
              for (int j = 0; j < 32; ++j)
                if (interior || fb + j < LN) d = fmaf(v[j], __ldg(P.wlast + fb + j), d);
              if (ts) dotb += d; else dota += d;
            } else {
#pragma unroll
              for (int g = 0; g < 4; ++g) store_group_hi(smem, ts ? OFF_ALO : OFF_AHI, fb + 8 * g, row, &v[8 * g]);
            }
          }
          if (need_store) signal_block(kb);
        }
        if (rank == 0 && warp == 4) TL_MARK(8 + m * 4 + 3);
        free_phase ^= (kc32_cur >= 16) ? 0xFFFFu : ((1u << kc32_cur) - 1u);
        if (last) {
          tc_fence_before();
          __syncwarp();
          if (lane == 0) mbar_arrive_cluster(FIN, 0);
          for (int ts = 0; ts < (has_b ? 2 : 1); ++ts) {
            part[row * 8 + pslot] = ts ? dotb : dota;
            epi_bar_sync();
            if (pslot == 0) {
              const float sv = row_sum8() * (1.f / sA) + __ldg(P.blast);
              float o = tanhf(sv);
              if (P.use_tanh) o = tanhf(o);
              float oc = o;
              if (io.clamp_dist > 0.f) oc = fminf(fmaxf(o, -io.clamp_dist), io.clamp_dist);
              const bool ok = ts ? okb : oka;
              if (ok && io.sdf) io.sdf[ts ? grb : gra] = oc;
              if (ok && !(fabsf(o) > io.screen_thresh)) near_flag[ts] = 1u;
            }
            epi_bar_sync();
          }
          if (ew == 0 && lane == 0) {
            for (int ts = 0; ts < (has_b ? 2 : 1); ++ts) {
              const bool fail = near_flag[ts] != 0u;
              if (fail) { fail_words[(i + ts) >> 5] |= 1u << ((i + ts) & 31); near_flag[ts] = 0u; }
              const int64_t r0 = row0_of(ts ? tb : ta) + rank * 64;
              if (io.seg_approx && r0 < n1) io.seg_approx[r0 >> 6] = fail ? 0 : 1;
              ++n_tiles_1pass;
            }
          }
        }
      }
    };

    for (int phase = 0; phase < 2; ++phase) {
    int i = next_tile(phase, -1);
    prefetch_points(phase, i);
    start_layer0(phase, i, 0);
    while (i >= 0) {
      const int64_t t = tile_of(i);
      const int inext = next_tile(phase, i);
      if (MODE == 0 && phase == 0 && i < c1) {
        run_pair(i, inext, i + 1 < c1);
        i = inext;
        continue;
      }
      const int64_t gr = row0_of(t) + rank * 64 + row;
      const bool row_ok = gr < lim_of(t);
      const int64_t slot = rec_slot(t);
      float dot = 0.f, rowscale = (MODE == 3) ? seed_scale : 0.f, dx = 0.f, dy = 0.f, dz = 0.f;
      uint32_t mk0s[2] = {0u, 0u};
      for (int m = m0; m < n_prog; ++m, ++G) {
        const uint32_t buf = G & 1;
        const bool fwd = m < n_mma;
        const bool fwd_last = (m == n_mma - 1);
        const bool prog_last = (m == n_prog - 1);
        const int LN = P.L[m].N, Lnh = P.L[m].nh, Lapp = P.L[m].app_xyz;
        const float cscale = P.L[m].inv_scale;
        const float* Lbias = P.L[m].bias;
        const int kc32_cur = P.L[m].kc32;
        auto wait_half = [&](int h) {
          const int bi = 2 * buf + h;
          mbar_wait(D_FULL(buf, h), (d_phase >> bi) & 1);
          d_phase ^= (1u << bi);
          tc_fence_after();
        };
        auto wait_free = [&](int kb) {
          if (kb < kc32_cur) mbar_wait(A_FREE(kb), (free_phase >> kb) & 1);
        };
        constexpr bool EARLY0 = (MODE == 0);
        if (prog_last) prefetch_points(phase, inext);
        if (prog_last && !EARLY0) for (int h = 0; h < Lnh; ++h) wait_half(h);
#ifdef DIST_TC_TIMELINE
        const bool dbg_rec = io.dbg_out && cluster_id == 0 && rank == 0 && warp == 4 && lane == 0 && t == cluster_id + n_clusters;
#else
        const bool dbg_rec = false;
#endif
        if (prog_last && !EARLY0) {
          mk0s[0] = mk[0][0]; mk0s[1] = mk[0][1];
          start_layer0(phase, inext, 0);
        }
        const int kblocks_next = prog_last ? 0 : P.L[m + 1].kc32;
        const int mask_layer = fwd ? (m + 1) : (2 * n_mma - m - 1);
        for (int h = 0; h < Lnh; ++h) {
          const int kb = 8 * h + 4 * q + ch;
          const int fb = 32 * kb;
          bool need_store = false, process = false;
          if (fwd && !fwd_last) { need_store = kb < kblocks_next; process = need_store; }
          else if (fwd_last) { process = fb < LN; }
          else if (!prog_last) { need_store = kb < kblocks_next; process = need_store || (Lapp && fb < LN + 3 && fb + 32 > LN); }
          else { process = fb < LN + 3 * Lapp; }
          if (EARLY0 && prog_last && h == Lnh - 1) start_layer0(phase, inext, kc32_cur);
          if (!prog_last || EARLY0) wait_half(h);
          if (!process) continue;
          if (dbg_rec && h == 0) io.dbg_out[8 + m * 4 + 2] = clock64();
          float v[32];
          tmem_ld32(tmem + lane_base + buf * 256 + h * 128 + 32 * ch, v);
          const bool interior = (fb + 32 <= LN);
          if (fwd) {
            uint32_t mb = 0;
            if (interior) {
#pragma unroll
              for (int j4 = 0; j4 < 8; ++j4) {
                const float4 b4 = __ldg(reinterpret_cast<const float4*>(Lbias + fb) + j4);
                const float bb[4] = {b4.x, b4.y, b4.z, b4.w};
#pragma unroll
                for (int e = 0; e < 4; ++e) {
                  const int j = 4 * j4 + e;
                  const float a = fmaf(v[j], cscale, bb[e]);
                  if (MODE != 0 || rec_on) mb |= (a > 0.f) ? (1u << j) : 0u;
                  v[j] = fmaxf(a, 0.f);
                }
              }
            } else {
#pragma unroll
              for (int j = 0; j < 32; ++j) {
                const int f = fb + j;
                float a = 0.f;
                if (f < LN) {
                  a = fmaf(v[j], cscale, __ldg(Lbias + f));
                  if (a > 0.f) mb |= 1u << j; else a = 0.f;
                } else if (Lapp && f < LN + 3) {
                  a = ((f == LN) ? px : ((f == LN + 1) ? py : pz)) * sA;
                }
                v[j] = a;
              }
            }
            if (MODE != 0) mk[m + 1][h] = mb;
            if (MODE == 0 && slot >= 0) io.mask_buf[((size_t)(m + 1) * 16 + kb) * io.mask_cap + slot] = mb;
            if (fwd_last) {
              if (interior) {
#pragma unroll
                for (int j4 = 0; j4 < 8; ++j4) {
                  const float4 w4 = __ldg(reinterpret_cast<const float4*>(P.wlast + fb) + j4);
                  dot = fmaf(v[4 * j4], w4.x, dot); dot = fmaf(v[4 * j4 + 1], w4.y, dot);
                  dot = fmaf(v[4 * j4 + 2], w4.z, dot); dot = fmaf(v[4 * j4 + 3], w4.w, dot);
                }
              } else {
#pragma unroll
                for (int j = 0; j < 32; ++j)
                  if (fb + j < LN) dot = fmaf(v[j], __ldg(P.wlast + fb + j), dot);
              }
            } else if (need_store) {
              wait_free(kb);
#pragma unroll
              for (int g = 0; g < 4; ++g) store_group(smem, fb + 8 * g, row, &v[8 * g]);
              signal_block(kb);
            }
          } else {
            const uint32_t mb = (mask_layer == 0 && prog_last) ? mk0s[h] : mk[mask_layer][h];
            if (interior) {
#pragma unroll
              for (int j = 0; j < 32; ++j) v[j] = ((mb >> j) & 1u) ? v[j] * cscale : 0.f;
            } else {
#pragma unroll
              for (int j = 0; j < 32; ++j) {
                const int f = fb + j;
                const float g = v[j] * cscale;
                float d = 0.f;
                if (f < LN) d = ((mb >> j) & 1u) ? g : 0.f;
                else if (Lapp && f < LN + 3) { if (f == LN) dx += g; else if (f == LN + 1) dy += g; else dz += g; }
                v[j] = d;
              }
            }
            if (prog_last) {
              if (interior) {
#pragma unroll
                for (int j4 = 0; j4 < 8; ++j4) {
                  const float4 wx = __ldg(reinterpret_cast<const float4*>(P.w0 + fb) + j4);
                  const float4 wy = __ldg(reinterpret_cast<const float4*>(P.w0 + P.N0p4 + fb) + j4);
                  const float4 wz = __ldg(reinterpret_cast<const float4*>(P.w0 + 2 * P.N0p4 + fb) + j4);
                  const int j = 4 * j4;
                  dx = fmaf(v[j], wx.x, dx); dx = fmaf(v[j + 1], wx.y, dx); dx = fmaf(v[j + 2], wx.z, dx); dx = fmaf(v[j + 3], wx.w, dx);
                  dy = fmaf(v[j], wy.x, dy); dy = fmaf(v[j + 1], wy.y, dy); dy = fmaf(v[j + 2], wy.z, dy); dy = fmaf(v[j + 3], wy.w, dy);
                  dz = fmaf(v[j], wz.x, dz); dz = fmaf(v[j + 1], wz.y, dz); dz = fmaf(v[j + 2], wz.z, dz); dz = fmaf(v[j + 3], wz.w, dz);
                }
              } else {
#pragma unroll
                for (int j = 0; j < 32; ++j) {
                  const int f = fb + j;
                  if (f < LN) {
                    dx = fmaf(v[j], __ldg(P.w0 + f), dx);
                    dy = fmaf(v[j], __ldg(P.w0 + P.N0p4 + f), dy);
                    dz = fmaf(v[j], __ldg(P.w0 + 2 * P.N0p4 + f), dz);
                  }
                }
              }
            } else if (need_store) {
              wait_free(kb);
#pragma unroll
              for (int g = 0; g < 4; ++g) store_group(smem, fb + 8 * g, row, &v[8 * g]);
              signal_block(kb);
            }
            if ((MODE == 2 || MODE == 3) && (prog_last || m == P.acc_l_prog)) {
#pragma unroll
              for (int j = 0; j < 32; ++j) v[j] *= rowscale;
              const float sres = colsum32(v);
              if (prog_last) acc0r[h] += sres; else acclr[h] += sres;
            }
          }
        }
        if (dbg_rec) io.dbg_out[8 + m * 4 + 3] = clock64();
        free_phase ^= (kc32_cur >= 16) ? 0xFFFFu : ((1u << kc32_cur) - 1u);
        if (fwd_last) {
          part[row * 8 + pslot] = dot;
          epi_bar_sync();
          if (pslot == 0) {
            const float s = row_sum8() * (1.f / sA) + __ldg(P.blast);
            float t1 = s, o = tanhf(s);
            if (P.use_tanh) { t1 = o; o = tanhf(o); }
            float oc = o;
            if (io.clamp_dist > 0.f) oc = fminf(fmaxf(o, -io.clamp_dist), io.clamp_dist);
            if (row_ok && io.sdf) io.sdf[gr] = oc;
            if (MODE != 0) {
              float d = 1.f - o * o;
              if (P.use_tanh) d *= (1.f - t1 * t1);
              bool uc = io.clamp_dist > 0.f;
              if (MODE == 2 && io.use_clamp) uc = row_ok ? (io.use_clamp[gr] != 0) : false;
              if (uc && !(o >= -io.clamp_dist && o <= io.clamp_dist)) d = 0.f;
              float cf = 1.f;
              if (MODE == 2 && io.coef) cf = row_ok ? io.coef[gr] : 0.f;
              if (!row_ok) cf = 0.f;
              rowd[row] = d * cf;
            }
          }
          epi_bar_sync();
          if (MODE == 0 && ew == 0 && lane == 0) {
            if (io.seg_approx && row0_of(t) + rank * 64 < lim_of(t)) io.seg_approx[(row0_of(t) >> 6) + rank] = 0;
            ++n_tiles_3pass;
          }
          if (MODE != 0) {
            rowscale = rowd[row];
            const int kblocks = P.L[n_mma].kc32;
            for (int h = 0; h < Lnh; ++h) {
              const int kb = 8 * h + 4 * q + ch;
              if (kb >= kblocks) continue;
              const int f0 = 32 * kb;
              const uint32_t mb = mk[n_mma][h];
#pragma unroll
              for (int g = 0; g < 4; ++g) {
                float x[8];
#pragma unroll
                for (int e = 0; e < 8; ++e) {
                  const int f = f0 + 8 * g + e;
                  x[e] = (f < LN && ((mb >> (8 * g + e)) & 1u)) ? __ldg(P.wlast + f) * sD : 0.f;
                }
                store_group(smem, f0 + 8 * g, row, x);
              }
              signal_block(kb);
            }
          }
        }
        if (prog_last) {
          tc_fence_before();
          __syncwarp();
          if (lane == 0) mbar_arrive_cluster(FIN, 0);
          if (MODE != 0) {
            float res[3];
#pragma unroll
            for (int k = 0; k < 3; ++k) {
              part[row * 8 + pslot] = (k == 0) ? dx : ((k == 1) ? dy : dz);
              epi_bar_sync();
              res[k] = row_sum8();
              epi_bar_sync();
            }
            if (pslot == 0 && row_ok && io.grad) {
              const float rs = rowscale * (1.f / sD);
              io.grad[gr * 3] = res[0] * rs; io.grad[gr * 3 + 1] = res[1] * rs; io.grad[gr * 3 + 2] = res[2] * rs;
            }
          }
        }
      }
      i = inext;
    }
      if (phase == 0) {
        if (!screening) break;
        cluster_sync_all();
      }
    }
    if (io.tile_counters && rank == 0 && ew == 0 && lane == 0) {
      if (MODE != 0) n_tiles_3pass = (MODE == 3 ? 1u : 2u) * (unsigned)cnt;
      if (n_tiles_1pass) atomicAdd(io.tile_counters, (unsigned long long)n_tiles_1pass);
      if (n_tiles_3pass) atomicAdd(io.tile_counters + 1, (unsigned long long)n_tiles_3pass);
    }
    if (MODE == 2 || MODE == 3) {
#pragma unroll
      for (int h = 0; h < 2; ++h) {
        const int f = 32 * (8 * h + 4 * q + ch) + lane;
        if (io.acc0 && f < P.N0 && acc0r[h] != 0.f) atomicAdd(io.acc0 + f, acc0r[h] * (1.f / sD));
        if (io.accl && P.acc_l_prog >= 0 && f < P.accl_N && acclr[h] != 0.f) atomicAdd(io.accl + f, acclr[h] * (1.f / sD));
      }
    }
  }
  if (io.dbg_out && blockIdx.x == 0 && tid == 0) {
    long long t1; asm volatile("mov.u64 %0, %%globaltimer;" : "=l"(t1));
    io.dbg_out[0] = clock64() - dbg_c0; io.dbg_out[1] = t1 - dbg_t0;
  }
  tc_fence_before();
  __syncthreads();
  cluster_sync_all();
  if (warp == 2) asm volatile("tcgen05.dealloc.cta_group::2.sync.aligned.b32 %0, %1;" ::"r"(tmem), "r"(512) : "memory");
}

typedef CUresult (*EncodeFn)(CUtensorMap*, CUtensorMapDataType, cuuint32_t, void*, const cuuint64_t*, const cuuint64_t*,
                             const cuuint32_t*, const cuuint32_t*, CUtensorMapInterleave, CUtensorMapSwizzle,
                             CUtensorMapL2promotion, CUtensorMapFloatOOBfill);

EncodeFn get_encode() {
  static EncodeFn fn = nullptr;
  static bool tried = false;
  if (!tried) {
    tried = true;
    cudaDriverEntryPointQueryResult q;
    void* p = nullptr;
    if (cudaGetDriverEntryPoint("cuTensorMapEncodeTiled", &p, cudaEnableDefault, &q) == cudaSuccess) fn = (EncodeFn)p;
  }
  return fn;
}

}

int mlp_tc_launch(const dist_net_t* net, const NetDev& nd, int mode, const MlpArgs& a, cudaStream_t stream) {
  DIST_REQUIRE(mode >= 0 && mode <= 3, "tensor-core engine: bad mode %d", mode);
  DIST_REQUIRE(mode != 3 || (a.slots && a.sdf_in && a.mask_buf && a.mask_cap > 0), "tensor-core engine: mode 3 needs the mask cache");
  DIST_REQUIRE(net->tc_blob && net->tc_scale, "tensor-core engine: operands not prepared (tc.prepare)");
  const int nl = nd.n_layers;
  DIST_REQUIRE(nl >= 4 && nl <= 10, "tensor-core engine: %d layers unsupported", nl);
  if (a.n_host <= 0 && !a.n_dev && a.n2_host <= 0 && !a.n2_dev) return DIST_OK;
  EncodeFn encode = get_encode();
  if (!encode) { set_error("cuTensorMapEncodeTiled not available"); return DIST_E_UNSUPPORTED; }

  TcParams P;
  memset(&P, 0, sizeof(P));
  P.n_mma = nl - 2;
  P.n_prog = (mode == 0) ? P.n_mma : 2 * P.n_mma;
  P.acc_l_prog = -1;
  int stage = 0;
  for (int m = 0; m < P.n_mma; ++m) {
    const int l = m + 1;
    LayerTC& L = P.L[m];
    L.kc32 = round_up(nd.K[l], 64) / 32;
    L.nh = (nd.N[l] + 255) / 256;
    L.stage_base = stage;
    stage += L.kc32 * L.nh;
    L.N = nd.N[l];
    L.app_xyz = (l + 1 == nd.latent_in) ? 1 : 0;
    L.inv_scale = net->tc_scale[m];
    L.bias = net->tc_bias[l];
    DIST_REQUIRE(L.bias != nullptr, "tensor-core engine: scaled bias missing for layer %d", l);
    DIST_REQUIRE(nd.N[l] + 3 * L.app_xyz <= 256 * L.nh && nd.N[l] <= 512, "tensor-core engine: layer %d width unsupported", l);
  }
  for (int j = 0; j < P.n_mma; ++j) {
    const int l = P.n_mma - j;
    LayerTC& L = P.L[P.n_mma + j];
    L.kc32 = round_up(nd.N[l], 64) / 32;
    L.nh = (nd.K[l] + 255) / 256;
    L.stage_base = stage;
    stage += L.kc32 * L.nh;
    L.N = nd.N[l - 1];
    L.app_xyz = (l == nd.latent_in) ? 1 : 0;
    L.inv_scale = net->tc_scale[P.n_mma + j];
    L.bias = nullptr;
    if (l - 1 == nd.latent_in) P.acc_l_prog = P.n_mma + j;
  }
  DIST_REQUIRE((int64_t)stage * 2 * STAGE_BYTES == net->tc_blob_bytes, "tensor-core engine: operand blob size mismatch");
  P.accl_N = (nd.latent_in >= 0) ? nd.N[nd.latent_in] : 0;
  P.w0 = nd.Wt[0]; P.bias0 = nd.bias[0]; P.N0 = nd.N[0]; P.N0p4 = round_up(nd.N[0], 4);
  P.wlast = nd.W[nl - 1]; P.blast = nd.bias[nl - 1]; P.K_last = nd.K[nl - 1];
  P.use_tanh = nd.use_tanh; P.sA = 32.0f; P.sD = 256.0f;
  P.first_append = (nd.latent_in == 1) ? 1 : 0;
  { const char* e = getenv("DIST_TC_DEBUG"); P.dbg = e ? atoi(e) : 0; }

  TcIO io;
  io.points = a.points; io.n_host = a.n_host; io.n_dev = a.n_dev; io.clamp_dist = a.clamp_dist;
  io.sdf = a.sdf; io.grad = a.grad; io.coef = a.coef; io.use_clamp = a.use_clamp; io.acc0 = a.acc0; io.accl = a.accl;
  io.rows_evaluated = a.rows_evaluated;
  io.n2_host = a.n2_host; io.n2_dev = a.n2_dev; io.seg2_offset = a.seg2_offset;
  io.screen_seg1 = (mode == 0) ? a.screen_seg1 : 0;
  io.screen_thresh = a.screen_thresh; io.seg_approx = a.seg_approx;
  io.tile_counters = a.tile_counters;
  io.mask_buf = a.mask_buf; io.mask_cap = a.mask_cap; io.mask_base_host = a.mask_buf ? a.mask_base_host : -1;
  io.mask_base_dev = a.mask_base_dev; io.slots = a.slots; io.sdf_in = a.sdf_in;
  DIST_REQUIRE(!io.screen_seg1 || io.seg_approx != nullptr, "tensor-core engine: two-tier precision needs seg_approx");
  DIST_REQUIRE((a.n2_host == 0 && !a.n2_dev) || (a.seg2_offset % 128 == 0 && a.seg2_offset >= a.n_host),
               "tensor-core engine: the second row segment must start at a multiple of 128 behind the first");
  io.dbg_out = nullptr;
  static long long* dbg_buf = nullptr;
  if (P.dbg & 4) { if (!dbg_buf) { cudaMalloc(&dbg_buf, 4096); cudaMemset(dbg_buf, 0, 4096); } io.dbg_out = dbg_buf; }

  static const int boxrow = [] { const char* e = getenv("DIST_TC_BOXROW"); int v = e ? atoi(e) : 128;
                                 return (v == 128 || v == 256 || v == 512) ? v : 128; }();
  P.stage_rows = STAGE_BYTES / boxrow;
  CUtensorMap tmap;
  const cuuint64_t rows = (cuuint64_t)(net->tc_blob_bytes / boxrow);
  const cuuint64_t gdim[2] = {(cuuint64_t)(boxrow / 2), rows};
  const cuuint64_t gstr[1] = {(cuuint64_t)boxrow};
  const cuuint32_t box[2] = {(cuuint32_t)(boxrow / 2), (cuuint32_t)(STAGE_BYTES / boxrow)};
  const cuuint32_t estr[2] = {1, 1};
  CUresult cr = encode(&tmap, CU_TENSOR_MAP_DATA_TYPE_FLOAT16, 2, const_cast<void*>(net->tc_blob), gdim, gstr, box, estr,
                       CU_TENSOR_MAP_INTERLEAVE_NONE, CU_TENSOR_MAP_SWIZZLE_NONE, CU_TENSOR_MAP_L2_PROMOTION_L2_256B,
                       CU_TENSOR_MAP_FLOAT_OOB_FILL_NONE);
  if (cr != CUDA_SUCCESS) { set_error("cuTensorMapEncodeTiled failed (%d)", (int)cr); return DIST_E_CUDA; }
  CUtensorMap tmap_hi;
  const cuuint32_t box_hi[2] = {(cuuint32_t)(boxrow / 2), (cuuint32_t)(STAGE_BYTES / 2 / boxrow)};
  cr = encode(&tmap_hi, CU_TENSOR_MAP_DATA_TYPE_FLOAT16, 2, const_cast<void*>(net->tc_blob), gdim, gstr, box_hi, estr,
              CU_TENSOR_MAP_INTERLEAVE_NONE, CU_TENSOR_MAP_SWIZZLE_NONE, CU_TENSOR_MAP_L2_PROMOTION_L2_256B,
              CU_TENSOR_MAP_FLOAT_OOB_FILL_NONE);
  if (cr != CUDA_SUCCESS) { set_error("cuTensorMapEncodeTiled (hi box) failed (%d)", (int)cr); return DIST_E_CUDA; }

  static bool attr_done_dev[64] = {false};
  int cur_dev = 0;
  cudaGetDevice(&cur_dev);
  bool& attr_done = attr_done_dev[cur_dev & 63];
  if (!attr_done) {
    DIST_CHECK_CUDA(cudaFuncSetAttribute(mlp_tc_kernel<0>, cudaFuncAttributeMaxDynamicSharedMemorySize, SMEM_BYTES));
    DIST_CHECK_CUDA(cudaFuncSetAttribute(mlp_tc_kernel<1>, cudaFuncAttributeMaxDynamicSharedMemorySize, SMEM_BYTES));
    DIST_CHECK_CUDA(cudaFuncSetAttribute(mlp_tc_kernel<2>, cudaFuncAttributeMaxDynamicSharedMemorySize, SMEM_BYTES));
    DIST_CHECK_CUDA(cudaFuncSetAttribute(mlp_tc_kernel<3>, cudaFuncAttributeMaxDynamicSharedMemorySize, SMEM_BYTES));
    attr_done = true;
  }
  const int64_t tiles = (a.n_host + 127) / 128 + (a.n2_host + 127) / 128;
  int clusters = num_sms() / 2;
  if (tiles < clusters) clusters = (int)tiles;
  if (clusters < 1) clusters = 1;
  if (mode == 0) { mlp_tc_kernel<0><<<clusters * 2, NTHREADS, SMEM_BYTES, stream>>>(tmap, tmap_hi, P, io); }
  else if (mode == 1) { mlp_tc_kernel<1><<<clusters * 2, NTHREADS, SMEM_BYTES, stream>>>(tmap, tmap_hi, P, io); }
  else if (mode == 2) { mlp_tc_kernel<2><<<clusters * 2, NTHREADS, SMEM_BYTES, stream>>>(tmap, tmap_hi, P, io); }
  else { mlp_tc_kernel<3><<<clusters * 2, NTHREADS, SMEM_BYTES, stream>>>(tmap, tmap_hi, P, io); }
  count_launch();
  DIST_CHECK_CUDA(cudaGetLastError());
  if (P.dbg & 4) {
    long long h[2] = {0, 0};
    cudaStreamSynchronize(stream);
    cudaMemcpy(h, dbg_buf, 16, cudaMemcpyDeviceToHost);
    fprintf(stderr, "[tc dbg] mode %d: %lld cycles, %lld ns -> %.3f GHz\n", mode, h[0], h[1], h[1] ? (double)h[0] / h[1] : 0.0);
#ifdef DIST_TC_TIMELINE
    {
      long long ev[256];
      cudaMemcpy(ev, dbg_buf, 2048, cudaMemcpyDeviceToHost);
      const long long t0 = ev[8];
      fprintf(stderr, "[tc dbg] previous tile: last MMA issue at %lld (relative to this tile's first MMA)\n", ev[200] - t0);
      long long wt[64];
      cudaMemcpy(wt, dbg_buf + 256, sizeof(wt), cudaMemcpyDeviceToHost);
      for (int m = 0; m < P.n_prog; ++m)
        fprintf(stderr, "[tc dbg] layer %2d: mma start %7lld  issue end %7lld | epi start %7lld  epi end %7lld | issuer waited for A %6lld, for W %6lld\n",
                m, ev[8 + m * 4] - t0, ev[8 + m * 4 + 1] - t0, ev[8 + m * 4 + 2] - t0, ev[8 + m * 4 + 3] - t0, wt[2 * m], wt[2 * m + 1]);
      cudaMemset(dbg_buf + 256, 0, sizeof(wt));
    }
#endif
  }
  return DIST_OK;
}

}
```

### dist-renderer_b200/renderer.py

```python
import os

import numpy as np
import torch

from . import _abi
from .functional import resolve_engine, DEFAULT_ENGINE
from .plan import plan_for

_MARCH = {"trivial": _abi.MARCH_TRIVIAL, "trivial_non_parallel": _abi.MARCH_TRIVIAL,
          "recursive": _abi.MARCH_RECURSIVE, "pyramid_recursive": _abi.MARCH_PYRAMID}


def _stream(device=None):
    return torch.cuda.current_stream(device).cuda_stream


class _RenderDepthFn(torch.autograd.Function):

    @staticmethod
    def forward(ctx, latent, R, T, ren, opts):
        with torch.cuda.device(ren.device):
            return _RenderDepthFn._forward(ctx, latent, R, T, ren, opts)

    @staticmethod
    def _forward(ctx, latent, R, T, ren, opts):
        lib, st = _abi.lib(), _stream(ren.device)
        plan = ren.plan
        plan.refresh()
        dev = ren.device
        P, B = ren.P, ren.buffer_size
        engine = resolve_engine(plan, opts["engine"])
        net, engine, _keep = plan.net_for(latent, engine, st)
        Rd = R.detach().float().contiguous()
        if Rd.shape != ((3, 3) if ren.n_views == 1 and R.dim() == 2 else (ren.n_views, 3, 3)):
            raise ValueError("R must be (3,3), or (n_views,3,3) on a multi-view renderer")
        cam_pos = ren.get_camera_location(Rd, T.detach().float()).contiguous()
        cam = ren._c_camera(Rd, cam_pos, opts["use_transform"])
        mp = _abi.March(ren.march_step, B, _MARCH[opts["kind"]], 1 if opts["kind"] != "pyramid_recursive" else 0,
                        ren.ray_marching_ratio, ren.threshold, float(opts["clamp_dist"]), opts["replay"])
        pyr = opts["kind"] == "pyramid_recursive"
        if pyr:
            mp.coarse_steps[0], mp.coarse_steps[1] = ren._coarse_steps()
        mp.cam_grad_levels = opts["cam_levels"]
        screen = plan.tc.get("screen") if (engine == _abi.ENGINE_TC and plan.tc is not None and ren.screen) else None
        if screen:
            mp.screen, mp.screen_margin = 1, screen["margin"]
            mp.screen_tpred, mp.screen_ext_margin = ren.screen_tpred, ren.screen_ext_margin
        f32 = dict(device=dev, dtype=torch.float32)
        saved = {
            "flags": torch.empty(P, device=dev, dtype=torch.uint8), "nreal": torch.empty(P, device=dev, dtype=torch.int32),
            "top_sdf": torch.empty(B, P, **f32), "top_pt": torch.empty(B, 3, P, **f32),
            "top_zafter": torch.empty(B, P, **f32), "top_zgen": torch.empty(B, P, **f32),
            "sdf_origin": torch.empty(1, **f32), "dist": torch.empty(P, **f32),
            "top_lvl": torch.empty(B, P, device=dev, dtype=torch.uint8),
        }
        scr = ren._scratch(pyramid=pyr)
        mask_cap = 0
        if screen and ren.mask_cache and (opts["want_depth_grad"] or opts["want_mask_grad"]):
            mask_cap = (int(ren.mask_rows_per_ray * P) + 127) // 128 * 128
            saved["mask_buf"] = torch.empty(16 * (plan.n_layers - 1) * mask_cap, device=dev, dtype=torch.int32)
            saved["top_slot"] = torch.empty(B, P, device=dev, dtype=torch.int32)
        ws = _abi.Workspace()
        for name in _abi.WS_FIELDS:
            if name == "mask_cap":
                continue
            t = saved.get(name, scr.get(name))
            setattr(ws, name, t.data_ptr() if t is not None else None)
        ws.mask_cap = mask_cap
        ws.tile_counters = ren.tile_counters.data_ptr()
        Zdepth = torch.empty(P, **f32)
        mask = torch.empty(P, device=dev, dtype=torch.uint8)
        min_sdf = torch.empty(P, **f32)
        _abi.check(lib.dist_render_depth_fwd(net, engine, cam, mp, ws, _abi.ptr(Zdepth), _abi.ptr(mask),
                                             _abi.ptr(min_sdf), _abi.ptr(ren.rows_evaluated), st))
        ren._last_counts = scr["view_stat"]
        ctx.ren, ctx.opts, ctx.engine, ctx.mp, ctx.mask_cap = ren, opts, engine, mp, mask_cap
        ctx.saved = saved
        ctx.save_for_backward(latent, Rd, T.detach().float())
        hit = saved["flags"].bitwise_and(1).bool()
        ctx.mark_non_differentiable(mask, hit)
        return Zdepth, mask, min_sdf, hit

    @staticmethod
    def backward(ctx, gZ, _gmask, gM, _ghit):
        with torch.cuda.device(ctx.ren.device):
            return _RenderDepthFn._backward(ctx, gZ, gM)

    @staticmethod
    def _backward(ctx, gZ, gM):
        latent, Rd, Td = ctx.saved_tensors
        ren, opts, lib, st = ctx.ren, ctx.opts, _abi.lib(), _stream(ctx.ren.device)
        plan, dev, P, B = ren.plan, ren.device, ren.P, ren.buffer_size
        net, eng_b, _keep = plan.net_for(latent, ctx.engine, st)
        cam_pos = ren.get_camera_location(Rd, Td).contiguous()
        cam = ren._c_camera(Rd, cam_pos, opts["use_transform"])
        V, Pv = ren.n_views, ren.Pv
        scr = ren._scratch()
        ws = _abi.Workspace()
        for name in _abi.WS_FIELDS:
            if name == "mask_cap":
                continue
            t = ctx.saved.get(name, scr.get(name))
            setattr(ws, name, t.data_ptr() if t is not None else None)
        ws.mask_cap = ctx.mask_cap
        pyr = opts["kind"] == "pyramid_recursive"
        gZ = gZ.contiguous().float() if (gZ is not None and opts["want_depth_grad"]) else None
        gM = gM.contiguous().float() if (gM is not None and opts["want_mask_grad"]) else None
        want_cam = opts["cam_levels"] != 0 and (ctx.needs_input_grad[1] or ctx.needs_input_grad[2])
        f32 = dict(device=dev, dtype=torch.float32)
        acc0 = torch.zeros(plan.bias[0].numel(), **f32)
        accl = torch.zeros(plan.bias[plan.latent_in].numel(), **f32) if plan.latent_in >= 0 else None
        d_cam = torch.zeros(V, 3, **f32) if want_cam else None
        d_ray = torch.zeros(3, P, **f32) if want_cam else None
        n_coarse = V * sum(g[0].shape[1] for g in ren._coarse_homo()) if (want_cam and pyr) else 0
        d_ray_c = torch.zeros(3 * n_coarse, **f32) if n_coarse else None
        g_lat = g_R = g_T = None
        if gZ is not None or gM is not None:
            s_row, s_pts, s_coef, s_dpts, s_cnt = scr["b_row"], scr["b_pts"], scr["b_coef"], scr["b_dpts"], scr["b_cnt"]
            _abi.check(lib.dist_render_depth_bwd(net, eng_b, cam, ctx.mp, ws, _abi.ptr(gZ), _abi.ptr(gM),
                                                 _abi.ptr(acc0), _abi.ptr(accl), _abi.ptr(d_cam), _abi.ptr(d_ray),
                                                 _abi.ptr(d_ray_c), _abi.ptr(s_row), _abi.ptr(s_pts), _abi.ptr(s_coef), None,
                                                 _abi.ptr(s_dpts), _abi.ptr(s_cnt), _abi.ptr(ren.rows_grad), st))
            if ctx.needs_input_grad[0] and latent is not None:
                g_lat = plan.latent_grad(acc0, accl).reshape(latent.shape).to(latent.dtype)
            if want_cam:
                with torch.enable_grad():
                    Rg, Tg = Rd.clone().requires_grad_(True), Td.clone().requires_grad_(True)
                    c = ren.get_camera_location(Rg, Tg)

                    def per_view(g, n):
                        return g.reshape(3, n) if Rg.dim() == 2 else g.reshape(3, V, n).permute(1, 0, 2)
                    outs, gouts = [c, ren.get_camera_rays(Rg)], [d_cam.reshape(c.shape), per_view(d_ray, Pv)]
                    if d_ray_c is not None:
                        off = 0
                        for (homo,) in ren._coarse_homo():
                            n_l = homo.shape[1]
                            outs.append(ren.get_camera_rays(Rg, homo=homo))
                            gouts.append(per_view(d_ray_c[off:off + 3 * V * n_l], n_l))
                            off += 3 * V * n_l
                    g_R, g_T = torch.autograd.grad(outs, [Rg, Tg], gouts, allow_unused=True)
        return g_lat, g_R, g_T, None, None


class SDFRenderer(object):
    def __init__(self, decoder, intrinsic, img_hw=None, transform_matrix=None, march_step=50, buffer_size=5,
                 ray_marching_ratio=1.5, use_depth2normal=False, max_sample_dist=0.2, radius=1.0, threshold=5e-5,
                 scale_list=[4, 2, 1], march_step_list=[3, 3, -1], use_gpu=True, is_eval=True, engine=None,
                 rows=None, screen=None, screen_tpred=0.30, screen_ext_margin=0.04, mask_cache=None, mask_rows_per_ray=9.0):
        self.decoder = decoder
        if use_gpu and torch.cuda.device_count() == 0:
            raise ValueError('No GPU device found.')
        if not use_gpu:
            raise RuntimeError("dist-renderer_b200 has no CPU path: use_gpu=False is not supported")
        p = next(self.decoder.parameters())
        if not p.is_cuda:
            raise ValueError("the decoder must be on a CUDA device (no CPU path)")
        self.device = p.device
        if is_eval:
            self.decoder.eval()
        if not (1 <= buffer_size <= _abi.MAX_BUFFER):
            raise NotImplementedError("buffer_size must be in [1, %d]" % _abi.MAX_BUFFER)
        self.march_step, self.buffer_size = int(march_step), int(buffer_size)
        self.max_sample_dist = max_sample_dist
        self.ray_marching_ratio = float(ray_marching_ratio)
        self.use_depth2normal = use_depth2normal
        self.radius, self.threshold = float(radius), float(threshold)
        self.scale_list, self.march_step_list = scale_list, march_step_list
        self.engine = engine or DEFAULT_ENGINE
        if type(intrinsic) == torch.Tensor:
            intrinsic = intrinsic.detach().cpu().numpy()
        self.intrinsic = np.asarray(intrinsic, dtype=np.float64)
        if img_hw is None:
            img_hw = (int(self.intrinsic[1, 2] * 2), int(self.intrinsic[0, 2] * 2))
        self.img_hw = (int(img_hw[0]), int(img_hw[1]))
        h, w = self.img_hw
        self.rows = (0, 1, h, 1) if rows is None else (tuple(int(v) for v in rows) + (1,))[:4]
        row0, step, n_rows, grp = self.rows
        if not (0 <= row0 and step >= 1 and n_rows >= 1 and grp >= 1 and
                row0 + ((n_rows - 1) // grp) * step + (n_rows - 1) % grp < h):
            raise ValueError("rows=(row0,row_step,n_rows[,row_group]) outside the image")
        self.full_image = (row0 == 0 and step == grp and n_rows == h)
        self.local_hw = (n_rows, w)
        self.n_views = 1
        self.Pv = n_rows * w
        self.P = self.Pv
        self.K = torch.from_numpy(self.intrinsic).float().to(self.device)
        self.K_inv = torch.from_numpy(np.linalg.inv(self.intrinsic)).float().to(self.device)
        if transform_matrix is None:
            transform_matrix = np.array([[1., 0., 0.], [0., 0., -1.], [0., 1., 0.]])
        transform_matrix = np.asarray(transform_matrix, dtype=np.float64)
        if transform_matrix.shape != (3, 3):
            raise NotImplementedError("only 3x3 transform_matrix is supported (renderer.py:116 is dead code upstream)")
        self.transform_matrix = torch.from_numpy(transform_matrix).float().to(self.device)
        self.plan = plan_for(decoder)
        self.rows_evaluated = torch.zeros(1, device=self.device, dtype=torch.int64)
        self.rows_grad = torch.zeros(2, device=self.device, dtype=torch.int64)
        self.tile_counters = torch.zeros(2, device=self.device, dtype=torch.int64)
        self.screen = (os.environ.get("DIST_SCREEN", "1") != "0") if screen is None else bool(screen)
        self.screen_tpred = float(os.environ.get("DIST_SCREEN_TPRED", screen_tpred))
        self.screen_ext_margin = float(os.environ.get("DIST_SCREEN_EXT", screen_ext_margin))
        self.mask_cache = (os.environ.get("DIST_MASK_CACHE", "1") != "0") if mask_cache is None else bool(mask_cache)
        self.mask_rows_per_ray = float(mask_rows_per_ray)
        self._homo_calib = None
        self._calib_map = None
        self._scr = None
        self._last_counts = None

    def get_intrinsic(self):
        return self.intrinsic

    def get_threshold(self):
        return self.threshold

    def get_img_hw(self):
        return self.img_hw

    @property
    def homo_calib(self):
        if self._homo_calib is None:
            w = self.img_hw[1]
            ys = self._image_rows(torch.arange(self.rows[2], device=self.device)).float()
            xs = torch.arange(w, device=self.device).float()
            Y, X = torch.meshgrid(ys, xs, indexing="ij")
            homo = torch.stack([X.reshape(-1), Y.reshape(-1), torch.ones(self.Pv, device=self.device)], 0)
            self._homo_calib = torch.matmul(self.K_inv, homo)
        return self._homo_calib

    @property
    def calib_map(self):
        if self._calib_map is None:
            self._calib_map = self.normalize_vectors(self.homo_calib)[2, :]
        return self._calib_map

    def normalize_vectors(self, x):
        return x.div(torch.norm(x, p=2, dim=0).expand_as(x) + 1e-12)

    def get_camera_location(self, R, T):
        if R.dim() == 3:
            return torch.stack([self.get_camera_location(R[v], T[v]) for v in range(R.shape[0])], 0)
        return torch.matmul(-R.transpose(1, 0), T[:, None]).squeeze(1)

    def get_camera_rays(self, R, homo=None):
        if R.dim() == 3:
            return torch.stack([self.get_camera_rays(R[v], homo) for v in range(R.shape[0])], 0)
        return self.normalize_vectors(torch.matmul(R.transpose(1, 0), self.homo_calib if homo is None else homo))

    def transform_points(self, points):
        return torch.matmul(self.transform_matrix, points)

    def inv_transform_points(self, points):
        return torch.matmul(self.transform_matrix.transpose(1, 0), points)

    def generate_point_samples(self, cam_pos, cam_rays, Zdepth, inv_transform=True, has_zdepth_grad=False):
        if not has_zdepth_grad:
            Zdepth = Zdepth.detach()
        if Zdepth.shape[0] == 0:
            raise ValueError('No valid depth.')
        points = cam_rays * Zdepth[None, :] + cam_pos[:, None]
        if inv_transform:
            points = self.inv_transform_points(points)
        if not points.requires_grad:
            points.requires_grad = True
        return points

    def get_distance_from_origin(self, cam_pos, cam_rays):
        if cam_rays.dim() == 3:
            return torch.stack([self.get_distance_from_origin(cam_pos[v], cam_rays[v]) for v in range(cam_rays.shape[0])], 0)
        ptq = (cam_pos[:, None] * cam_rays).sum(0)
        return torch.norm(cam_pos[:, None] - ptq[None, :] * cam_rays, p=2, dim=0)

    def _image_rows(self, local_rows):
        row0, step, _, grp = self.rows
        return row0 + (local_rows // grp) * step + local_rows % grp

    def _transform_host(self):
        tm = self.transform_matrix
        key = (id(tm), tm._version)
        if getattr(self, "_tm_host_key", None) != key:
            self._tm_host = tm.detach().cpu().numpy().astype(np.float32).reshape(-1)
            self._tm_host_key = key
        return self._tm_host

    def _c_camera(self, R, cam_pos, use_transform=True):
        cam = _abi.Camera()
        Kinv = np.linalg.inv(self.intrinsic).astype(np.float32).reshape(-1)
        Mn = self._transform_host()
        M = Mn if use_transform else np.eye(3).reshape(-1)
        for i in range(9):
            cam.Kinv[i], cam.M[i], cam.Mn[i] = float(Kinv[i]), float(M[i]), float(Mn[i])
        cam._keep = (R, cam_pos)
        cam.R, cam.cam_pos = R.data_ptr(), cam_pos.data_ptr()
        cam.width, cam.height = self.img_hw[1], self.img_hw[0]
        cam.row0, cam.row_step, cam.n_rows, cam.row_group = self.rows
        cam.radius = self.radius
        cam.n_views = self.n_views
        return cam

    def _coarse_steps(self):
        if list(self.scale_list) != [4, 2, 1] or len(self.march_step_list) != 3 or self.march_step_list[2] != -1:
            raise NotImplementedError("pyramid_recursive is implemented for scale_list=[4,2,1], march_step_list=[a,b,-1]")
        a, b = int(self.march_step_list[0]), int(self.march_step_list[1])
        if not (1 <= a <= 3 and 1 <= b <= 3 and a + b < self.march_step):
            raise NotImplementedError("pyramid_recursive: coarse step counts must be in [1,3]")
        return a, b

    def _coarse_dims(self):
        h, w = self.local_hw
        h1, w1 = (h + 1) // 2, (w + 1) // 2
        h2, w2 = (h1 + 1) // 2, (w1 + 1) // 2
        return (h1, w1), (h2, w2)

    def _coarse_homo(self):
        if getattr(self, "_chomo", None) is None:
            res = []
            for (hh, ww), scale in zip(self._coarse_dims(), (2, 4)):
                ys = self._image_rows(scale * torch.arange(hh, device=self.device)).float() + (scale - 1) / 2
                xs = scale * torch.arange(ww, device=self.device).float() + (scale - 1) / 2
                Y, X = torch.meshgrid(ys, xs, indexing="ij")
                homo = torch.stack([X.reshape(-1), Y.reshape(-1), torch.ones(hh * ww, device=self.device)], 0)
                res.append((torch.matmul(self.K_inv, homo),))
            self._chomo = res
        return self._chomo

    def _scratch(self, pyramid=False):
        if pyramid and self._scr is not None and self._scr.get("pyr_f") is None:
            (h1, w1), (h2, w2) = self._coarse_dims()
            npc = (h1 * w1 + h2 * w2) * self.n_views
            self._scr["pyr_f"] = torch.empty(23 * npc, device=self.device, dtype=torch.float32)
            self._scr["pyr_i"] = torch.empty(4 * npc + 8, device=self.device, dtype=torch.int32)
            self._scr["pyr_b"] = torch.empty(npc, device=self.device, dtype=torch.uint8)
        if self._scr is None:
            P, dev = self.P, self.device
            SEG = (P + 1 + 127) // 128 * 128
            f32 = dict(device=dev, dtype=torch.float32)
            i32 = dict(device=dev, dtype=torch.int32)
            self._scr = {
                "ray": torch.empty(3, P, **f32), "entry": torch.empty(P, **f32), "exit_": torch.empty(P, **f32),
                "entry0": torch.empty(P, **f32), "pyr_f": None, "pyr_i": None, "pyr_b": None,
                "z": torch.empty(P, **f32), "list_a": torch.empty(2 * SEG, **i32), "list_b": torch.empty(2 * SEG, **i32),
                "pts": torch.empty(2, 2 * SEG, 3, **f32), "sdf": torch.empty(2 * SEG, **f32),
                "counts": torch.empty(2 * (self.march_step + 2), **i32),
                "view_stat": torch.zeros(self.n_views, 4, **i32),
                "n_idx": torch.empty(P, **i32), "n_pts": torch.empty(P, 3, **f32), "n_grad": torch.empty(P, 3, **f32),
                "n_cnt": torch.empty(1, **i32),
                "b_row": torch.empty(P * self.buffer_size, **i32), "b_pts": torch.empty(P * self.buffer_size, 3, **f32),
                "b_coef": torch.empty(P * self.buffer_size, **f32), "b_dpts": torch.empty(P * self.buffer_size, 3, **f32),
                "b_cnt": torch.empty(1, **i32),
                "seg_approx": torch.zeros(2 * SEG // 64, device=dev, dtype=torch.uint8), "sprev": torch.empty(P, **f32),
            }
            n_b = P * self.buffer_size
            self._scr.update(mask_base=torch.zeros(self.march_step + 3, **i32), bm_row=torch.empty(n_b, **i32),
                             bm_slot=torch.empty(n_b, **i32), bm_sdf=torch.empty(n_b, **f32), bm_coef=torch.empty(n_b, **f32),
                             bm_dpts=torch.empty(n_b, 3, **f32), bm_cnt=torch.empty(1, **i32))
            self._scr.update(rq_idx=self._scr["b_row"], rq_pts=self._scr["b_pts"], rq_sdf=self._scr["b_coef"],
                             rq_cnt=self._scr["b_cnt"])
            if pyramid:
                return self._scratch(pyramid=True)
        return self._scr

    def _raise_if_empty(self, stat=None):
        stat = self._last_counts.cpu() if stat is None else stat
        if int(stat[:, 3].max()) != 0:
            raise FloatingPointError("non-finite sdf during the march: the decoder's activations overflow the fp16 "
                                     "operands of the tensor-core engine for this latent; use engine='simt'")
        if int(stat[:, 0].min()) == 0:
            raise ValueError('No valid depth.')

    def reset_row_counter(self):
        self.rows_evaluated.zero_()
        self.rows_grad.zero_()
        self.tile_counters.zero_()

    def flops_per_row(self):
        return 2 * sum(k * n for k, n in zip(self.plan.K, self.plan.N))

    def render_depth(self, latent, R, T, clamp_dist=0.1, sample_index_type='min_abs', profile=False, no_grad=False,
                     no_grad_depth=False, no_grad_mask=False, no_grad_camera=False, ray_marching_type='recursive',
                     use_transform=True, check_empty=True):
        if no_grad:
            no_grad_depth, no_grad_mask, no_grad_camera = True, True, True
        ngd_views = None
        if isinstance(no_grad_depth, (list, tuple)):
            if len(no_grad_depth) != self.n_views or self.n_views > 31:
                raise ValueError("no_grad_depth needs one flag per view (at most 31 views)")
            ngd_views = [bool(f) for f in no_grad_depth]
            no_grad_depth = all(ngd_views)
        if sample_index_type != 'min_abs':
            raise NotImplementedError("sample_index_type='%s' is not implemented (only 'min_abs')" % sample_index_type)
        if ray_marching_type == 'pyramid_recursive':
            self._coarse_steps()
            if not self.full_image and self.rows[3] % 4 != 0:
                raise NotImplementedError("pyramid_recursive on a row band needs bands of 4-row groups "
                                          "(rows=(row0,row_step,n_rows,4)); single-row bands use 'recursive'")
        if ray_marching_type not in _MARCH:
            raise ValueError('Error! Invalid type of ray marching: {}.'.format(ray_marching_type))
        any_grad = torch.is_grad_enabled() and any(t is not None and t.requires_grad for t in (latent, R, T))
        cam_levels = 3
        if no_grad_camera:
            cam_levels = {"recursive": 0, "pyramid_recursive": 2}.get(ray_marching_type, 3)
        opts = dict(kind=ray_marching_type, clamp_dist=clamp_dist, use_transform=use_transform, engine=self.engine,
                    want_depth_grad=any_grad and not no_grad_depth, want_mask_grad=any_grad and not no_grad_mask,
                    cam_levels=cam_levels if any_grad else 0,
                    replay=(sum(1 << v for v, f in enumerate(ngd_views) if not f) if ngd_views is not None
                            else (0 if no_grad_depth else -2147483648)))
        Zdepth, mask, min_sdf, hit = _RenderDepthFn.apply(latent, R, T, self, opts)
        if check_empty:
            self._raise_if_empty()
        if torch.is_grad_enabled() and (R.requires_grad or T.requires_grad):
            cam_pos = self.get_camera_location(R, T)
            d = self.get_distance_from_origin(cam_pos, self.get_camera_rays(R)).reshape(-1)
            min_sdf = torch.where(hit, min_sdf, d + self.threshold - self.radius)
        if no_grad_depth:
            Zdepth = Zdepth.detach()
        elif ngd_views is not None and any(ngd_views):
            Zv = Zdepth.reshape(self.n_views, self.Pv)
            Zdepth = torch.stack([Zv[v].detach() if f else Zv[v] for v, f in enumerate(ngd_views)], 0).reshape(-1)
        if no_grad_mask and not (R.requires_grad or T.requires_grad):
            min_sdf = min_sdf.detach()
        return Zdepth, mask.bool(), min_sdf

    def render_normal(self, latent, R, T, Zdepth, valid_mask, clamp_dist=0.1, MAX_POINTS=100000, no_grad=False,
                      normalize=True, use_transform=True):
        with torch.cuda.device(self.device):
            Znormal, n_idx = self._render_normal_raw(latent, R, T, Zdepth, valid_mask, clamp_dist, normalize,
                                                     use_transform)
            want_graph = (not normalize) and (not no_grad) and torch.is_grad_enabled() and \
                any(t is not None and t.requires_grad for t in (latent, R, T))
            if not want_graph:
                return Znormal
            from .functional import decode_sdf
            idx = torch.nonzero(valid_mask.reshape(-1).bool()).reshape(-1)
            if idx.numel() == 0:
                return Znormal
            v = idx // self.Pv if R.dim() == 3 else None
            cam_pos, cam_rays = self.get_camera_location(R, T), self.get_camera_rays(R)
            if v is None:
                pts = cam_rays[:, idx] * Zdepth.detach()[idx][None, :] + cam_pos[:, None]
            else:
                pts = cam_rays[v, :, idx - v * self.Pv].t() * Zdepth.detach()[idx][None, :] + cam_pos[v].t()
            if use_transform:
                pts = self.inv_transform_points(pts)
            o = decode_sdf(self.decoder, latent, pts.t(), clamp_dist=None, engine=self.engine).squeeze(-1)

            def dchain(x):
                if self.plan.use_tanh:
                    return (1 - x * x) * (1 - torch.atanh(x) ** 2)
                return 1 - x * x
            factor = dchain(o) / dchain(o.detach())
            scale = torch.ones(self.P, device=self.device, dtype=torch.float32).index_copy(0, idx, factor)
            return Znormal * scale[None, :]

    def _render_normal_raw(self, latent, R, T, Zdepth, valid_mask, clamp_dist, normalize, use_transform):
        lib, st = _abi.lib(), _stream(self.device)
        plan = self.plan
        plan.refresh()
        engine = resolve_engine(plan, self.engine)
        net, engine, _keep = plan.net_for(latent, engine, st)
        Rd = R.detach().float().contiguous()
        cam_pos = self.get_camera_location(Rd, T.detach().float()).contiguous()
        cam = self._c_camera(Rd, cam_pos, use_transform)
        scr = self._scratch()
        Zd = Zdepth.detach().float().contiguous()
        m8 = valid_mask.detach().to(torch.uint8).contiguous()
        Znormal = torch.empty(3, self.P, device=self.device, dtype=torch.float32)
        _abi.check(lib.dist_render_normal_fwd(net, engine, cam, _abi.ptr(Zd), _abi.ptr(m8), float(clamp_dist),
                                              1 if normalize else 0, _abi.ptr(Znormal), _abi.ptr(scr["n_idx"]),
                                              _abi.ptr(scr["n_pts"]), _abi.ptr(scr["n_grad"]), _abi.ptr(scr["n_cnt"]),
                                              _abi.ptr(self.rows_grad), st))
        return Znormal, scr["n_idx"]

    def render(self, latent, R, T, clamp_dist=0.1, sample_index_type='min_abs', profile=False, no_grad=False,
               no_grad_depth=False, no_grad_normal=False, no_grad_mask=False, no_grad_camera=False,
               normalize_normal=True, use_transform=True, ray_marching_type='pyramid_recursive',
               num_forward_sampling=0, check_empty=True):
        if no_grad:
            no_grad_depth, no_grad_normal, no_grad_mask, no_grad_camera = True, True, True, True
        h, w = self.local_hw
        Zdepth, valid_mask, min_abs_query = self.render_depth(
            latent, R, T, clamp_dist=clamp_dist, sample_index_type=sample_index_type, profile=profile, no_grad=no_grad,
            no_grad_depth=no_grad_depth, no_grad_mask=no_grad_mask, no_grad_camera=no_grad_camera,
            ray_marching_type=ray_marching_type, use_transform=use_transform, check_empty=False)
        V, stacked = self.n_views, R.dim() == 3
        calib = self.calib_map.repeat(V) if stacked else self.calib_map
        depth = torch.where(valid_mask, Zdepth * calib, torch.full_like(Zdepth, 1e11))
        if self.use_depth2normal:
            from .render_utils import depth2normal
            fx, fy = np.float32(self.intrinsic[0, 0]), np.float32(self.intrinsic[1, 1])
            dmap = depth.reshape((V, h, w) if stacked else (h, w))
            normal = torch.stack([depth2normal(dmap[v], fx, fy) for v in range(V)], 0) if stacked \
                else depth2normal(dmap, fx, fy)
            out = (dmap, normal, valid_mask.reshape(dmap.shape).type(torch.uint8), min_abs_query.reshape(dmap.shape))
            if num_forward_sampling != 0:
                if stacked:
                    raise NotImplementedError("forward sampling is not available on the multi-view march")
                inside = self.forward_sampling(latent, R, T, Zdepth, valid_mask, clamp_dist=clamp_dist,
                                               num_forward_sampling=num_forward_sampling, use_transform=use_transform)
                out = out + (inside.reshape(h, w, num_forward_sampling),)
            if check_empty:
                self._raise_if_empty()
            return out
        normal = self.render_normal(latent, R, T, Zdepth, valid_mask, clamp_dist=clamp_dist, no_grad=no_grad_normal,
                                    normalize=normalize_normal, use_transform=use_transform)
        if stacked:
            if num_forward_sampling != 0:
                raise NotImplementedError("forward sampling is not available on the multi-view march")
            Rn, n3 = R, normal.reshape(3, V, -1)
            normal = torch.stack([torch.matmul(Rn[v], n3[:, v].contiguous()) for v in range(V)], 0)
            normal = torch.cat([normal[:, :1] * (-1), normal[:, 1:]], 1).reshape(V, 3, h, w).permute(0, 2, 3, 1)
            out = (depth.reshape(V, h, w), normal, valid_mask.reshape(V, h, w).type(torch.uint8),
                   min_abs_query.reshape(V, h, w))
            if check_empty:
                self._raise_if_empty()
            return out
        normal = torch.matmul(R, normal)
        normal = torch.cat([normal[:1] * (-1), normal[1:]], 0)
        normal = normal.reshape(3, h, w).permute(1, 2, 0)
        out = (depth.reshape(h, w), normal, valid_mask.reshape(h, w).type(torch.uint8), min_abs_query.reshape(h, w))
        if num_forward_sampling != 0:
            inside = self.forward_sampling(latent, R, T, Zdepth, valid_mask, clamp_dist=clamp_dist,
                                           num_forward_sampling=num_forward_sampling, use_transform=use_transform)
            out = out + (inside.reshape(h, w, num_forward_sampling),)
        if check_empty:
            self._raise_if_empty()
        return out

    def _fused_child(self, V):
        import copy
        cache = self.__dict__.setdefault("_fused", {})
        child = cache.get(V)
        if child is None:
            child = copy.copy(self)
            child.n_views, child.P = V, V * self.Pv
            child._scr, child._last_counts, child._slots, child._fused = None, None, None, {}
            cache[V] = child
        return child

    def _view_slots(self, n):
        import copy
        slots = getattr(self, "_slots", None) or []
        while len(slots) < n:
            child = copy.copy(self)
            child._scr, child._last_counts, child._slots, child._fused = None, None, None, {}
            slots.append((torch.cuda.Stream(device=self.device), child))
        self._slots = slots
        return slots[:n]

    def render_views(self, latent, Rs, Ts, fused=True, n_streams=1, **kw):
        check_empty = kw.pop("check_empty", True)
        V = len(Rs)
        if V == 0 or len(Ts) != V:
            raise ValueError("render_views needs V >= 1 rotations and as many translations")
        if fused and kw.get("num_forward_sampling", 0) == 0:
            R = Rs if torch.is_tensor(Rs) else torch.stack(list(Rs), 0)
            T = Ts if torch.is_tensor(Ts) else torch.stack(list(Ts), 0)
            return self._fused_child(V).render(latent, R, T, check_empty=check_empty, **kw)
        main = torch.cuda.current_stream(self.device)
        _ = self.calib_map, self._coarse_homo()
        self.plan.refresh()
        self.plan.net_for(latent, resolve_engine(self.plan, self.engine), main.cuda_stream)
        n_streams = max(1, min(int(n_streams), V))
        slots = self._view_slots(n_streams)
        side = n_streams > 1
        n_valid = torch.empty(V, device=self.device, dtype=torch.int32)
        if side:
            for st, _ in slots:
                st.wait_stream(main)
        outs = []
        for v in range(V):
            st, child = slots[v % n_streams]
            with torch.cuda.stream(st if side else main):
                o = child.render(latent, Rs[v], Ts[v], check_empty=False, **kw)
                n_valid[v:v + 1].copy_(child._last_counts[:, 0])
            outs.append(o)
        if side:
            for st, _ in slots:
                main.wait_stream(st)
            for o in outs:
                for t in o:
                    t.record_stream(main)
        res = tuple(torch.stack([o[i] for o in outs], 0) for i in range(len(outs[0])))
        if check_empty and min(n_valid.tolist()) == 0:
            raise ValueError('No valid depth.')
        return res

    def forward_sampling(self, latent, R, T, Zdepth, valid_mask, clamp_dist=0.1, num_forward_sampling=1, no_grad=False,
                         use_transform=True):
        from .functional import decode_sdf
        assert num_forward_sampling > 0
        cam_pos = self.get_camera_location(R, T)
        cam_rays = self.get_camera_rays(R)
        inside = torch.zeros(self.P, num_forward_sampling, device=self.device, dtype=torch.float32)
        valid_mask = valid_mask.bool()
        idx = torch.nonzero(valid_mask).reshape(-1)
        if idx.numel() == 0:
            return inside
        rays_v, z_v = cam_rays[:, idx], Zdepth[idx]
        cols = []
        for i in range(num_forward_sampling):
            grid = 0.5 * clamp_dist * (i + 1) / num_forward_sampling
            pts = self.generate_point_samples(cam_pos, rays_v, z_v + grid, has_zdepth_grad=False, inv_transform=use_transform)
            sdf = decode_sdf(self.decoder, latent, pts.transpose(1, 0), clamp_dist=None, no_grad=no_grad,
                             engine=self.engine).squeeze(-1)
            cols.append(sdf[:, None] + grid)
        return inside.index_copy(0, idx, torch.cat(cols, 1))

    def render_silhouette(self, latent, R, T, **kw):
        h, w = self.local_hw
        _, valid_mask, min_abs_query = self.render_depth(latent, R, T, **kw)
        return valid_mask.reshape(h, w).type(torch.uint8), min_abs_query.reshape(h, w)
```

Baseline: 8.977 million.

## Fuse march tail steps into persistent tensor-core MLP kernel with on-chip ray ring

When few rays remain alive in the sphere march, the tensor-core MLP kernel switches to a persistent tail mode. It evaluates the SDF, performs the march update (z advance, top-k insert, next point) in its epilogue warps, and feeds surviving rays back through a cluster-shared ring buffer. A device flag then makes the later per-step MLP and march-update launches exit immediately. The aim is to remove many small launches and global round trips over the long, low-occupancy tail of marching, at the cost of extra cluster synchronisation, more complex control flow, and thresholds tuned by wave counts.

```diff
diff --git a/dist-renderer_b200/csrc/common.cuh b/dist-renderer_b200/csrc/common.cuh
--- a/dist-renderer_b200/csrc/common.cuh
+++ b/dist-renderer_b200/csrc/common.cuh
@@ -38,6 +38,8 @@
 
 int make_netdev(const dist_net_t* net, NetDev* out);
 
+struct MarchTail;
+
 struct MlpArgs {
   const float* points;
   int64_t n_host;
@@ -63,6 +65,7 @@
   const int32_t* mask_base_dev;
   const int32_t* slots;
   const float* sdf_in;
+  const MarchTail* tail;
 };
 int mlp_simt_launch(const NetDev& net, int mode, const MlpArgs& a, cudaStream_t stream);
 int mlp_tc_launch(const dist_net_t* net, const NetDev& nd, int mode, const MlpArgs& a, cudaStream_t stream);
diff --git a/dist-renderer_b200/csrc/march.cu b/dist-renderer_b200/csrc/march.cu
--- a/dist-renderer_b200/csrc/march.cu
+++ b/dist-renderer_b200/csrc/march.cu
@@ -1,30 +1,17 @@
 #include <cuda_runtime.h>
 #include <math.h>
+#include <stdio.h>
+#include <stdlib.h>
 #include <string.h>
 #include "common.cuh"
+#include "march_row.cuh"
 
 namespace dist {
 namespace {
 
-struct Cam {
-  float Kinv[9], M[9], Mn[9];
-  const float* R;
-  const float* c;
-  int W, H, row0, row_step, n_rows, row_group;
-  int n_views, Pv;
-  float radius;
-};
-
-enum { LVL_APPROX = 0x80, LVL_REQUERIED = 0x40 };
-enum { VS_LIVE0 = 0, VS_STEPS = 1, VS_MAXENTRY = 2, VS_NONFINITE = 3, VS_STRIDE = 4 };
-
 __device__ __forceinline__ void load_view(const Cam& cam, int v, float (&R)[9], float (&c)[3]) {
 #pragma unroll
   for (int i = 0; i < 9; ++i) R[i] = cam.R[9 * v + i];
-#pragma unroll
-  for (int i = 0; i < 3; ++i) c[i] = cam.c[3 * v + i];
-}
-__device__ __forceinline__ void load_view_pos(const Cam& cam, int v, float (&c)[3]) {
 #pragma unroll
   for (int i = 0; i < 3; ++i) c[i] = cam.c[3 * v + i];
 }
@@ -33,10 +20,6 @@
 __device__ __forceinline__ void view_atomic_add(int32_t* view_stat, int slot, int v) {
   const unsigned peers = __match_any_sync(0xffffffffu, v);
   if (v >= 0 && (int)(threadIdx.x & 31) == __ffs(peers) - 1) atomicAdd(view_stat + VS_STRIDE * v + slot, __popc(peers));
-}
-__device__ __forceinline__ void view_atomic_max(int32_t* view_stat, int slot, int v, int value) {
-  const unsigned peers = __match_any_sync(0xffffffffu, v);
-  if (v >= 0 && (int)(threadIdx.x & 31) == __ffs(peers) - 1) atomicMax(view_stat + VS_STRIDE * v + slot, value);
 }
 
 __device__ __forceinline__ int warp_append(int32_t* counter, bool pred) {
@@ -96,26 +79,6 @@
   ex = entry + chord;
 }
 
-__device__ __forceinline__ void topk_insert(const dist_workspace_t& ws, int P, int B, int lp, float sdf, float px, float py,
-                                            float pz, float zafter, float zgen, int lvl, int slot = -1) {
-  const float asdf = fabsf(sdf);
-  int pos = 0;
-  float worst = -1.f;
-  for (int b = 0; b < B; ++b) {
-    const float a = fabsf(ws.top_sdf[(size_t)b * P + lp]);
-    if (a >= worst) { worst = a; pos = b; }
-  }
-  if (!(asdf < worst)) return;
-  ws.top_sdf[(size_t)pos * P + lp] = sdf;
-  ws.top_zafter[(size_t)pos * P + lp] = zafter;
-  ws.top_zgen[(size_t)pos * P + lp] = zgen;
-  ws.top_lvl[(size_t)pos * P + lp] = (uint8_t)lvl;
-  if (ws.top_slot) ws.top_slot[(size_t)pos * P + lp] = slot;
-  ws.top_pt[((size_t)pos * 3 + 0) * P + lp] = px;
-  ws.top_pt[((size_t)pos * 3 + 1) * P + lp] = py;
-  ws.top_pt[((size_t)pos * 3 + 2) * P + lp] = pz;
-}
-
 struct Level {
   int w, h, Pv, P, scale;
   float *ray, *start, *z, *s_sdf, *s_pt, *s_zabs, *s_zgen;
@@ -124,17 +87,6 @@
   int32_t* count;
   int32_t* s_slot;
 };
-
-__device__ __forceinline__ void point_on_ray(const Cam& cam, const float (&c)[3], const float (&ray)[3], float depth,
-                                             float (&p)[3]) {
-  float q[3];
-#pragma unroll
-  for (int i = 0; i < 3; ++i) q[i] = ray[i] * depth + c[i];
-#pragma unroll
-  for (int i = 0; i < 3; ++i) p[i] = fmaf(cam.M[6 + i], q[2], fmaf(cam.M[3 + i], q[1], cam.M[i] * q[0]));
-}
-
-__device__ __forceinline__ float clampf(float v, float c) { return fminf(fmaxf(v, -c), c); }
 
 constexpr int BLK_W = 16, BLK_H = 8;
 __host__ __device__ inline int setup_threads_per_view(int W, int n_rows) {
@@ -317,6 +269,7 @@
 }
 
 __global__ void k_march_update(Cam cam, dist_march_t mp, dist_workspace_t ws, int step, int P) {
+  if (*march_tail_flag(ws, mp.march_step) != 0) return;
   const int SEG = seg_capacity(P);
   const int n1 = ws.counts[2 * step];
   const int n2 = (step == 0) ? 0 : ws.counts[2 * step + 1];
@@ -329,53 +282,28 @@
   if (step == 0 && blockIdx.x == 0 && threadIdx.x == 0) ws.sdf_origin[0] = ws.sdf[SEG];
   const bool mc = scr && ws.mask_buf != nullptr;
   const int mbase = mc ? ws.mask_base[step] : 0;
-  if (mc && blockIdx.x == 0 && threadIdx.x == 0)
-    ws.mask_base[step + 1] = mbase + (ws.counts[2 * step + 1] + 127) / 128 * 128;
-  const int B = mp.buffer_size;
-  const float far_thresh = mp.clamp_dist + mp.screen_margin;
+  if (mc && blockIdx.x == 0 && threadIdx.x == 0) {
+    const int next_base = mbase + (ws.counts[2 * step + 1] + 127) / 128 * 128;
+    ws.mask_base[step + 1] = next_base;
+    ws.mask_base[mp.march_step] = next_base;
+  }
   for (int base = blockIdx.x * blockDim.x; base < n; base += gridDim.x * blockDim.x) {
     const int j = base + threadIdx.x;
-    bool live = false, approx = false, pred_far = false;
+    bool live = false, pred_far = false;
     int lp = 0, v = -1;
-    float znew = 0.f, entry = 0.f;
+    float p[3] = {0.f, 0.f, 0.f};
     if (j < n) {
       const int i = (j < n1) ? j : SEG + (j - n1);
       lp = cur[i];
       v = lp / cam.Pv;
-      const float sdf = ws.sdf[i];
-      const float px = pts_cur[(size_t)i * 3], py = pts_cur[(size_t)i * 3 + 1], pz = pts_cur[(size_t)i * 3 + 2];
-      const float zc = ws.z[lp];
-      entry = ws.entry[lp];
-      znew = zc + clampf(sdf, mp.clamp_dist) * mp.ratio;
-      ws.z[lp] = znew;
-      ws.nreal[lp] = step + 1;
-      if (step == 0 && sdf > mp.threshold) ws.flags[lp] |= 2;
-      const float asdf = fabsf(sdf);
-      approx = scr && ws.seg_approx[i >> 6] != 0;
-      if (scr) {
-        const float ext = sdf + (sdf - ws.sprev[lp]);
-        pred_far = asdf > mp.screen_tpred ||
-                   (step >= 1 && asdf > far_thresh && fabsf(ext) > far_thresh + mp.screen_ext_margin && (ext > 0.f) == (sdf > 0.f));
-        ws.sprev[lp] = sdf;
-      }
-      if (!(asdf <= 1.0f)) atomicOr(ws.view_stat + VS_STRIDE * v + VS_NONFINITE, 1);
-      const float zstore = (mp.marching_type == DIST_MARCH_PYRAMID) ? (znew + entry) - ws.entry0[lp] : znew;
+      const bool approx = scr && ws.seg_approx[i >> 6] != 0;
       int slot = -1;
       if (mc && i >= SEG && (int64_t)mbase + (i - SEG) < ws.mask_cap) slot = mbase + (i - SEG);
-      topk_insert(ws, P, B, lp, sdf, px, py, pz, zstore, entry + zc, approx ? LVL_APPROX : 0, slot);
-      if (step + 1 < mp.march_step) {
-        if (mp.marching_type == DIST_MARCH_TRIVIAL) live = true;
-        else live = (znew + entry < ws.exit_[lp]) && (asdf >= mp.threshold);
-      }
+      live = march_row_update(cam, mp, ws, P, step, lp, ws.sdf[i], pts_cur[(size_t)i * 3], pts_cur[(size_t)i * 3 + 1],
+                              pts_cur[(size_t)i * 3 + 2], approx, slot, pred_far, p);
     }
     view_atomic_max(ws.view_stat, VS_STEPS, v, step + 1);
     const bool to1 = live && (!scr || pred_far), to2 = live && !to1;
-    float p[3] = {0.f, 0.f, 0.f};
-    if (live) {
-      float ray[3] = {ws.ray[lp], ws.ray[P + lp], ws.ray[2 * P + lp]}, c[3];
-      load_view_pos(cam, v, c);
-      point_on_ray(cam, c, ray, entry + znew, p);
-    }
     int idx, idx2;
     warp_append2(ws.counts + 2 * (step + 1), to1, to2, idx, idx2);
     if (idx2 >= 0) idx = SEG + idx2;
@@ -717,7 +645,7 @@
   DIST_CHECK_CUDA(cudaMemsetAsync(ws->view_stat, 0, sizeof(int32_t) * VS_STRIDE * cam.n_views, st));
   const int S_total = mp->march_step;
   const int tb = 256, gb = (P + tb - 1) / tb;
-  const bool scr = mp->screen != 0 && engine == DIST_ENGINE_TC;
+  const bool scr = (mp->screen & 1) && engine == DIST_ENGINE_TC;
   const int SEG = seg_capacity(P);
   dist_workspace_t wsv = *ws;
   if (scr) {
@@ -783,6 +711,17 @@
   k_append_origin<<<1, 1, 0, st>>>(*ws, SEG, (int)coarse_slots); count_launch();
   DIST_CHECK_CUDA(cudaGetLastError());
   const int gu = min(gb, 4 * num_sms());
+  MarchTail tail;
+  memset(&tail, 0, sizeof(tail));
+  tail.on = scr && (mp->screen & 2) ? 1 : 0;
+  tail.P = P; tail.cam = cam; tail.mp = *mp; tail.ws = *ws;
+  tail.flag = march_tail_flag(*ws, S);
+  tail.rows_waves = 6.f; tail.far_waves = 0.5f; tail.early_min = 64;
+  if (const char* e = getenv("DIST_MARCH_TAIL_WAVES")) {
+    float r = 0.f, f = 0.f;
+    int em = tail.early_min;
+    if (sscanf(e, "%f,%f,%d", &r, &f, &em) >= 2) { tail.rows_waves = r; tail.far_waves = f; tail.early_min = em; }
+  }
   for (int s = 0; s < S; ++s) {
     MlpArgs a{};
     a.points = ws->pts + (size_t)(s & 1) * (size_t)(2 * SEG) * 3;
@@ -792,6 +731,8 @@
     a.tile_counters = ws->tile_counters;
     if (scr) { a.screen_seg1 = 1; a.screen_thresh = mp->clamp_dist + mp->screen_margin; a.seg_approx = ws->seg_approx; }
     if (mc) { a.mask_buf = ws->mask_buf; a.mask_cap = ws->mask_cap; a.mask_base_dev = ws->mask_base + s; }
+    tail.step = s;
+    if (tail.on) a.tail = &tail;
     rc = mlp_launch(net, nd, engine, 0, a, st);
     if (rc) return rc;
     k_march_update<<<gu, tb, 0, st>>>(cam, *mp, *ws, s, P); count_launch();
diff --git a/dist-renderer_b200/csrc/march_row.cuh b/dist-renderer_b200/csrc/march_row.cuh
--- /dev/null
+++ b/dist-renderer_b200/csrc/march_row.cuh
@@ -0,0 +1,111 @@
+#pragma once
+#include <cuda_runtime.h>
+#include <math.h>
+#include "common.cuh"
+
+namespace dist {
+
+struct Cam {
+  float Kinv[9], M[9], Mn[9];
+  const float* R;
+  const float* c;
+  int W, H, row0, row_step, n_rows, row_group;
+  int n_views, Pv;
+  float radius;
+};
+
+enum { LVL_APPROX = 0x80, LVL_REQUERIED = 0x40 };
+enum { VS_LIVE0 = 0, VS_STEPS = 1, VS_MAXENTRY = 2, VS_NONFINITE = 3, VS_STRIDE = 4 };
+
+struct MarchTail {
+  int on;
+  int step;
+  int P;
+  float rows_waves;
+  float far_waves;
+  int early_min;
+  int32_t* flag;
+  Cam cam;
+  dist_march_t mp;
+  dist_workspace_t ws;
+};
+__host__ __device__ inline int32_t* march_tail_flag(const dist_workspace_t& ws, int S) { return ws.counts + 2 * S + 2; }
+
+__device__ __forceinline__ void load_view_pos(const Cam& cam, int v, float (&c)[3]) {
+#pragma unroll
+  for (int i = 0; i < 3; ++i) c[i] = cam.c[3 * v + i];
+}
+
+__device__ __forceinline__ void view_atomic_max(int32_t* view_stat, int slot, int v, int value) {
+  const unsigned peers = __match_any_sync(0xffffffffu, v);
+  const int mx = (int)__reduce_max_sync(peers, (unsigned)value);
+  if (v >= 0 && (int)(threadIdx.x & 31) == __ffs(peers) - 1) atomicMax(view_stat + VS_STRIDE * v + slot, mx);
+}
+
+__device__ __forceinline__ void point_on_ray(const Cam& cam, const float (&c)[3], const float (&ray)[3], float depth,
+                                             float (&p)[3]) {
+  float q[3];
+#pragma unroll
+  for (int i = 0; i < 3; ++i) q[i] = __fadd_rn(__fmul_rn(ray[i], depth), c[i]);
+#pragma unroll
+  for (int i = 0; i < 3; ++i) p[i] = fmaf(cam.M[6 + i], q[2], fmaf(cam.M[3 + i], q[1], __fmul_rn(cam.M[i], q[0])));
+}
+
+__device__ __forceinline__ float clampf(float v, float c) { return fminf(fmaxf(v, -c), c); }
+
+__device__ __forceinline__ void topk_insert(const dist_workspace_t& ws, int P, int B, int lp, float sdf, float px, float py,
+                                            float pz, float zafter, float zgen, int lvl, int slot = -1) {
+  const float asdf = fabsf(sdf);
+  int pos = 0;
+  float worst = -1.f;
+  for (int b = 0; b < B; ++b) {
+    const float a = fabsf(ws.top_sdf[(size_t)b * P + lp]);
+    if (a >= worst) { worst = a; pos = b; }
+  }
+  if (!(asdf < worst)) return;
+  ws.top_sdf[(size_t)pos * P + lp] = sdf;
+  ws.top_zafter[(size_t)pos * P + lp] = zafter;
+  ws.top_zgen[(size_t)pos * P + lp] = zgen;
+  ws.top_lvl[(size_t)pos * P + lp] = (uint8_t)lvl;
+  if (ws.top_slot) ws.top_slot[(size_t)pos * P + lp] = slot;
+  ws.top_pt[((size_t)pos * 3 + 0) * P + lp] = px;
+  ws.top_pt[((size_t)pos * 3 + 1) * P + lp] = py;
+  ws.top_pt[((size_t)pos * 3 + 2) * P + lp] = pz;
+}
+
+__device__ __forceinline__ bool march_row_update(const Cam& cam, const dist_march_t& mp, const dist_workspace_t& ws, int P,
+                                                 int step, int lp, float sdf, float px, float py, float pz, bool approx,
+                                                 int slot, bool& pred_far, float (&pn)[3]) {
+  const int v = lp / cam.Pv;
+  const float zc = ws.z[lp];
+  const float entry = ws.entry[lp];
+  const float znew = __fadd_rn(zc, __fmul_rn(clampf(sdf, mp.clamp_dist), mp.ratio));
+  ws.z[lp] = znew;
+  ws.nreal[lp] = step + 1;
+  if (step == 0 && sdf > mp.threshold) ws.flags[lp] |= 2;
+  const float asdf = fabsf(sdf);
+  pred_far = false;
+  if (ws.seg_approx) {
+    const float far_thresh = mp.clamp_dist + mp.screen_margin;
+    const float ext = sdf + (sdf - ws.sprev[lp]);
+    pred_far = asdf > mp.screen_tpred ||
+               (step >= 1 && asdf > far_thresh && fabsf(ext) > far_thresh + mp.screen_ext_margin && (ext > 0.f) == (sdf > 0.f));
+    ws.sprev[lp] = sdf;
+  }
+  if (!(asdf <= 1.0f)) atomicOr(ws.view_stat + VS_STRIDE * v + VS_NONFINITE, 1);
+  const float zstore = (mp.marching_type == DIST_MARCH_PYRAMID) ? (znew + entry) - ws.entry0[lp] : znew;
+  topk_insert(ws, P, mp.buffer_size, lp, sdf, px, py, pz, zstore, entry + zc, approx ? LVL_APPROX : 0, slot);
+  bool live = false;
+  if (step + 1 < mp.march_step) {
+    if (mp.marching_type == DIST_MARCH_TRIVIAL) live = true;
+    else live = (znew + entry < ws.exit_[lp]) && (asdf >= mp.threshold);
+  }
+  if (live) {
+    float ray[3] = {ws.ray[lp], ws.ray[P + lp], ws.ray[2 * P + lp]}, c[3];
+    load_view_pos(cam, v, c);
+    point_on_ray(cam, c, ray, entry + znew, pn);
+  }
+  return live;
+}
+
+}
diff --git a/dist-renderer_b200/csrc/mlp_tc.cu b/dist-renderer_b200/csrc/mlp_tc.cu
--- a/dist-renderer_b200/csrc/mlp_tc.cu
+++ b/dist-renderer_b200/csrc/mlp_tc.cu
@@ -5,6 +5,7 @@
 #include <stdlib.h>
 #include <string.h>
 #include "common.cuh"
+#include "march_row.cuh"
 
 namespace dist {
 namespace {
@@ -78,6 +79,8 @@
   const int32_t* mask_base_dev;
   const int32_t* slots;
   const float* sdf_in;
+  MarchTail tail;
+  int64_t tail_rows_max, tail_far_max;
 };
 
 __device__ __forceinline__ uint32_t smem_u32(const void* p) { return (uint32_t)__cvta_generic_to_shared(p); }
@@ -112,6 +115,22 @@
   asm volatile("mapa.shared::cluster.u32 %0, %1, %2;" : "=r"(remote) : "r"(local_addr), "r"(rank));
   asm volatile("ld.shared::cluster.u32 %0, [%1];" : "=r"(v) : "r"(remote) : "memory");
   return v;
+}
+__device__ __forceinline__ void st_dsmem_u32(uint32_t local_addr, uint32_t rank, uint32_t v) {
+  uint32_t remote;
+  asm volatile("mapa.shared::cluster.u32 %0, %1, %2;" : "=r"(remote) : "r"(local_addr), "r"(rank));
+  asm volatile("st.shared::cluster.u32 [%0], %1;" ::"r"(remote), "r"(v) : "memory");
+}
+__device__ __forceinline__ void mbar_arrive_release_cluster(uint32_t bar_local, uint32_t rank) {
+  uint32_t remote;
+  asm volatile("mapa.shared::cluster.u32 %0, %1, %2;" : "=r"(remote) : "r"(bar_local), "r"(rank));
+  asm volatile("mbarrier.arrive.release.cluster.shared::cluster.b64 _, [%0];" ::"r"(remote) : "memory");
+}
+__device__ __forceinline__ void mbar_wait_acquire_cluster(uint32_t bar, uint32_t parity) {
+  asm volatile(
+      "{\n.reg .pred p;\nWAIT_%=:\n"
+      "mbarrier.try_wait.parity.acquire.cluster.shared::cta.b64 p, [%0], %1;\n"
+      "@p bra DONE_%=;\nbra WAIT_%=;\nDONE_%=:\n}\n" ::"r"(bar), "r"(parity) : "memory");
 }
 __device__ __forceinline__ uint64_t make_desc(uint32_t saddr, uint32_t lbo, uint32_t sbo) {
   uint64_t d = 0;
@@ -185,17 +204,21 @@
     const int64_t v0 = io.n_dev ? (int64_t)*io.n_dev : io.n_host;
     const int64_t v1 = io.n2_dev ? (int64_t)*io.n2_dev : io.n2_host;
     const int64_t v2 = (MODE == 0 && io.mask_buf) ? (io.mask_base_dev ? (int64_t)*io.mask_base_dev : io.mask_base_host) : -1;
-    hdr[0] = v0; hdr[1] = v1; hdr[2] = v2;
+    const int64_t v3 = (MODE == 0 && io.tail.on) ? (int64_t)*io.tail.flag : 0;
+    hdr[0] = v0; hdr[1] = v1; hdr[2] = v2; hdr[3] = v3;
   }
   __syncthreads();
+  if (MODE == 0 && io.tail.on && hdr[3] != 0 && hdr[3] != io.tail.step + 1) return;
   const int64_t n1 = hdr[0], n2 = hdr[1];
   const int64_t n = n1 + n2;
   if (n <= 0) return;
+  const bool tail = (MODE == 0) && io.tail.on && io.tail.step >= 1 && n <= io.tail_rows_max && n1 <= io.tail_far_max;
+  if (tail && blockIdx.x == 0 && threadIdx.x == 0) *io.tail.flag = io.tail.step + 1;
   const uint32_t rank = cluster_ctarank();
   const int tid = threadIdx.x, warp = tid >> 5, lane = tid & 31;
   const int cluster_id = blockIdx.x >> 1, n_clusters = gridDim.x >> 1;
   const int64_t tiles1 = (n1 + 127) / 128, n_tiles = tiles1 + (n2 + 127) / 128;
-  if ((blockIdx.x >> 1) >= n_tiles) return;
+  if (tail ? (int64_t)2 * cluster_id >= n : (blockIdx.x >> 1) >= n_tiles) return;
   auto row0_of = [&](int64_t t) -> int64_t { return (t < tiles1) ? t * 128 : io.seg2_offset + (t - tiles1) * 128; };
   auto lim_of = [&](int64_t t) -> int64_t { return (t < tiles1) ? n1 : io.seg2_offset + n2; };
   if (blockIdx.x == 0 && tid == 0 && io.rows_evaluated)
@@ -217,7 +240,7 @@
   const int m0 = (MODE == 3) ? P.n_mma : 0;
 
   const int cnt = (cluster_id < n_tiles) ? (int)((n_tiles - cluster_id + n_clusters - 1) / n_clusters) : 0;
-  const bool screening = (MODE == 0) && io.screen_seg1 != 0 && cnt <= 32 * FAIL_WORDS;
+  const bool screening = (MODE == 0) && !tail && io.screen_seg1 != 0 && cnt <= 32 * FAIL_WORDS;
   volatile uint32_t* near_flag = reinterpret_cast<volatile uint32_t*>(smem + OFF_FAIL);
   volatile uint32_t* fail_words = reinterpret_cast<volatile uint32_t*>(smem + OFF_FAIL + 16);
   const uint32_t fail_addr = sbase + OFF_FAIL + 16;
@@ -237,7 +260,23 @@
     return -1;
   };
 
+  const uint32_t DECIDED = bar0 + 8 * (2 * NST + 38), XE = bar0 + 8 * (2 * NST + 39), XL = bar0 + 8 * (2 * NST + 40);
+  volatile int32_t* tl = reinterpret_cast<volatile int32_t*>(smem + OFF_FAIL);
+  const int tl_cap = tail ? (int)(n / gridDim.x + ((int64_t)blockIdx.x < n % gridDim.x ? 1 : 0)) : 0;
+  const int tl_off = tail ? (int)(blockIdx.x * (n / gridDim.x) + min((int64_t)blockIdx.x, n % gridDim.x)) : 0;
+  const int tail_S = io.tail.mp.march_step;
+  const int tail_SEG2 = 2 * (int)io.seg2_offset;
+  int32_t* const ring_lp = tail ? ((io.tail.step & 1) ? io.tail.ws.list_a : io.tail.ws.list_b) : nullptr;
+  float* const ring_pts = tail ? io.tail.ws.pts + (size_t)((io.tail.step + 1) & 1) * (size_t)tail_SEG2 * 3 : nullptr;
+  auto tail_wait = [&](int k) -> int {
+    mbar_wait(DECIDED, (uint32_t)k & 1u);
+    return tl[4 + (k & 1)] ? k : -1;
+  };
+
   if (tid == 0) {
+    if (tail) {
+      mbar_init(DECIDED, 1); mbar_init(XE, 1); mbar_init(XL, 1);
+    }
     for (int s = 0; s < NST; ++s) { mbar_init(W_FULL(s), 1); mbar_init(W_EMPTY(s), 1); }
     for (int c = 0; c < 16; ++c) mbar_init(A_FULL(c), 4);
     for (int c = 0; c < 16; ++c) mbar_init(A_FREE(c), 1);
@@ -245,6 +284,7 @@
     mbar_init(FIN, 32);
     near_flag[0] = 0u; near_flag[1] = 0u;
     for (int w = 0; w < FAIL_WORDS; ++w) fail_words[w] = 0u;
+    if (tail) { tl[0] = 0; tl[1] = tl_cap; tl[2] = tl_cap; tl[3] = tl_off; }
     asm volatile("fence.mbarrier_init.release.cluster;" ::: "memory");
   }
   if (warp == 2) {
@@ -262,7 +302,7 @@
       uint32_t p_slot = 0, p_phase = 0;
       const uint32_t bar_leader_mask = 0xFEFFFFFFu;
       for (int phase = 0; phase < 2; ++phase) {
-        for (int i = next_tile(phase, -1); i >= 0; i = next_tile(phase, i)) {
+        for (int i = tail ? tail_wait(0) : next_tile(phase, -1); i >= 0; i = tail ? tail_wait(i + 1) : next_tile(phase, i)) {
           const bool exact = !(phase == 0 && i < c1);
           for (int m = m0; m < n_prog; ++m) {
             const int kc32 = P.L[m].kc32, sb = P.L[m].stage_base;
@@ -312,7 +352,7 @@
       uint32_t d_first = 1;
       bool prev_pair = false;
       for (int phase = 0; phase < 2; ++phase) {
-      for (int i = next_tile(phase, -1); i >= 0; i = next_tile(phase, i)) {
+      for (int i = tail ? tail_wait(0) : next_tile(phase, -1); i >= 0; i = tail ? tail_wait(i + 1) : next_tile(phase, i)) {
         const int64_t t = tile_of(i);
         const bool exact = !(phase == 0 && i < c1);
         const bool has_b = !exact && (i + 1 < c1);
@@ -601,13 +641,116 @@
         signal_block(kb);
       }
     };
+    int lp_nx = -1, lp_cur = -1;
+    float cx = 0.f, cy = 0.f, cz = 0.f, tail_o = 0.f;
+    uint32_t xe_ph = 0, xl_ph = 0;
+    const bool decider = (tid == 128);
+    auto tail_slot = [&](int k) -> int64_t {
+      const int p = k & 1, sb = tl[10 + p];
+      return (mask_base >= 0 && row < tl[6 + p] && sb >= 0 && (int64_t)sb + row < io.mask_cap) ? (int64_t)sb + row : -1;
+    };
+    auto tail_load = [&](int k) {
+      const int p = k & 1;
+      if (row < tl[6 + p]) {
+        const int e = tl_off + (tl[8 + p] + row) % (MODE == 0 ? tl_cap : 1);
+        lp_nx = ring_lp[e];
+        px = ring_pts[(size_t)e * 3]; py = ring_pts[(size_t)e * 3 + 1]; pz = ring_pts[(size_t)e * 3 + 2];
+      } else { lp_nx = -1; px = py = pz = 0.f; }
+    };
+    auto tail_pop = [&](int k) {
+      const int p = k & 1, head = tl[0], take = min(64, tl[1] - head);
+      tl[8 + p] = head; tl[6 + p] = take; tl[0] = head + take;
+      tl[10 + p] = (mask_base >= 0 && take > 0) ? atomicAdd(io.tail.ws.mask_base + tail_S, take) : -1;
+    };
+    auto tail_publish = [&](int k, bool go) {
+      tl[4 + (k & 1)] = go ? 1 : 0;
+      asm volatile("mbarrier.arrive.shared::cta.b64 _, [%0];" ::"r"(DECIDED) : "memory");
+    };
+    auto tail_start = [&]() -> int {
+      const int32_t* cur_lp = (io.tail.step & 1) ? io.tail.ws.list_b : io.tail.ws.list_a;
+      for (int k = tid - 128; k < tl_cap; k += 512) {
+        const int64_t j = (int64_t)blockIdx.x + (int64_t)k * gridDim.x;
+        const int64_t r = (j < n1) ? j : io.seg2_offset + (j - n1);
+        ring_lp[tl_off + k] = cur_lp[r];
+#pragma unroll
+        for (int c = 0; c < 3; ++c) ring_pts[(size_t)(tl_off + k) * 3 + c] = io.points[r * 3 + c];
+      }
+      __threadfence_block();
+      epi_bar_sync();
+      if (decider) { tail_pop(0); tail_publish(0, true); }
+      epi_bar_sync();
+      return 0;
+    };
+    auto tail_early = [&](int i) -> int {
+      if (decider) {
+        const int pend = tl[1] - tl[0], infl = tl[6 + (i & 1)];
+        st_dsmem_u32(smem_u32((const void*)&tl[12]), rank ^ 1u, (uint32_t)pend);
+        st_dsmem_u32(smem_u32((const void*)&tl[13]), rank ^ 1u, (uint32_t)infl);
+        mbar_arrive_release_cluster(XE, rank ^ 1u);
+        mbar_wait_acquire_cluster(XE, xe_ph); xe_ph ^= 1u;
+        const int pp = tl[12], pi = tl[13];
+        const int em = io.tail.early_min;
+        const bool early = (pend >= em || infl == 0) && (pp >= em || pi == 0) && pend + pp > 0;
+        tl[15] = early ? 1 : 0;
+        if (early) { tail_pop(i + 1); tail_publish(i + 1, true); }
+      }
+      epi_bar_sync();
+      return tl[15] ? i + 1 : -2;
+    };
+    auto tail_late = [&](int i) -> int {
+      if (decider) {
+        const int pend = tl[1] - tl[0];
+        st_dsmem_u32(smem_u32((const void*)&tl[14]), rank ^ 1u, (uint32_t)pend);
+        mbar_arrive_release_cluster(XL, rank ^ 1u);
+        mbar_wait_acquire_cluster(XL, xl_ph); xl_ph ^= 1u;
+        const bool go = pend + tl[14] > 0;
+        if (go) tail_pop(i + 1);
+        tail_publish(i + 1, go);
+      }
+      epi_bar_sync();
+      return tl[4 + ((i + 1) & 1)] ? i + 1 : -1;
+    };
+    auto tail_update = [&](int64_t slot_cur) {
+      if (warp == 4 || warp == 5) {
+        bool live = false, pred_far = false;
+        float pn[3] = {0.f, 0.f, 0.f};
+        int v = -1, step = 0;
+        if (lp_cur >= 0) {
+          step = io.tail.ws.nreal[lp_cur];
+          v = lp_cur / io.tail.cam.Pv;
+          live = march_row_update(io.tail.cam, io.tail.mp, io.tail.ws, io.tail.P, step, lp_cur, tail_o, cx, cy, cz, false,
+                                  (int)slot_cur, pred_far, pn);
+        }
+        view_atomic_max(io.tail.ws.view_stat, VS_STEPS, v, step + 1);
+        const unsigned m = __ballot_sync(0xffffffffu, live);
+        if (m) {
+          const int leader = __ffs(m) - 1;
+          int base = 0;
+          if (lane == leader) {
+            base = atomicAdd(const_cast<int32_t*>(&tl[1]), __popc(m));
+            if (io.rows_evaluated) atomicAdd(reinterpret_cast<unsigned long long*>(io.rows_evaluated), (unsigned long long)__popc(m));
+          }
+          base = __shfl_sync(0xffffffffu, base, leader);
+          if (live) {
+            const int e = tl_off + (base + __popc(m & ((1u << lane) - 1))) % (MODE == 0 ? tl_cap : 1);
+            ring_lp[e] = lp_cur;
+            ring_pts[(size_t)e * 3] = pn[0]; ring_pts[(size_t)e * 3 + 1] = pn[1]; ring_pts[(size_t)e * 3 + 2] = pn[2];
+          }
+        }
+      }
+      __threadfence_block();
+      epi_bar_sync();
+    };
+
     auto prefetch_points = [&](int phase, int inext) {
       if (inext < 0 || MODE == 3) return;
+      if (tail) { tail_load(inext); return; }
       if (phase == 0 && inext < c1) load_points_pair(inext); else load_point(tile_of(inext));
     };
     auto start_layer0 = [&](int phase, int inext, int guard_kc32) {
       if (inext < 0) return;
       if (MODE == 3) { seed(tile_of(inext)); return; }
+      if (tail) { layer0(tail_slot(inext), guard_kc32); return; }
       if (phase == 0 && inext < c1) layer0_pair(guard_kc32); else layer0(rec_slot(tile_of(inext)), guard_kc32);
     };
     auto run_pair = [&](int i, int inext, bool has_b) {
@@ -710,12 +853,12 @@
     };
 
     for (int phase = 0; phase < 2; ++phase) {
-    int i = next_tile(phase, -1);
+    int i = tail ? tail_start() : next_tile(phase, -1);
     prefetch_points(phase, i);
     start_layer0(phase, i, 0);
     while (i >= 0) {
       const int64_t t = tile_of(i);
-      const int inext = next_tile(phase, i);
+      int inext = tail ? -2 : next_tile(phase, i);
       if (MODE == 0 && phase == 0 && i < c1) {
         run_pair(i, inext, i + 1 < c1);
         i = inext;
@@ -723,7 +866,8 @@
       }
       const int64_t gr = row0_of(t) + rank * 64 + row;
       const bool row_ok = gr < lim_of(t);
-      const int64_t slot = rec_slot(t);
+      const int64_t slot = tail ? tail_slot(i) : rec_slot(t);
+      if (tail) { lp_cur = lp_nx; cx = px; cy = py; cz = pz; }
       float dot = 0.f, rowscale = (MODE == 3) ? seed_scale : 0.f, dx = 0.f, dy = 0.f, dz = 0.f;
       uint32_t mk0s[2] = {0u, 0u};
       for (int m = m0; m < n_prog; ++m, ++G) {
@@ -745,7 +889,10 @@
           if (kb < kc32_cur) mbar_wait(A_FREE(kb), (free_phase >> kb) & 1);
         };
         constexpr bool EARLY0 = (MODE == 0);
-        if (prog_last) prefetch_points(phase, inext);
+        if (prog_last) {
+          if (tail) inext = tail_early(i);
+          prefetch_points(phase, inext);
+        }
         if (prog_last && !EARLY0) for (int h = 0; h < Lnh; ++h) wait_half(h);
 #ifdef DIST_TC_TIMELINE
         const bool dbg_rec = io.dbg_out && cluster_id == 0 && rank == 0 && warp == 4 && lane == 0 && t == cluster_id + n_clusters;
@@ -887,7 +1034,8 @@
             if (P.use_tanh) { t1 = o; o = tanhf(o); }
             float oc = o;
             if (io.clamp_dist > 0.f) oc = fminf(fmaxf(o, -io.clamp_dist), io.clamp_dist);
-            if (row_ok && io.sdf) io.sdf[gr] = oc;
+            if (tail) tail_o = oc;
+            else if (row_ok && io.sdf) io.sdf[gr] = oc;
             if (MODE != 0) {
               float d = 1.f - o * o;
               if (P.use_tanh) d *= (1.f - t1 * t1);
@@ -902,7 +1050,7 @@
           }
           epi_bar_sync();
           if (MODE == 0 && ew == 0 && lane == 0) {
-            if (io.seg_approx && row0_of(t) + rank * 64 < lim_of(t)) io.seg_approx[(row0_of(t) >> 6) + rank] = 0;
+            if (io.seg_approx && !tail && row0_of(t) + rank * 64 < lim_of(t)) io.seg_approx[(row0_of(t) >> 6) + rank] = 0;
             ++n_tiles_3pass;
           }
           if (MODE != 0) {
@@ -931,6 +1079,13 @@
           tc_fence_before();
           __syncwarp();
           if (lane == 0) mbar_arrive_cluster(FIN, 0);
+          if (tail) {
+            tail_update(slot);
+            if (inext == -2) {
+              inext = tail_late(i);
+              if (inext >= 0) { tail_load(inext); layer0(tail_slot(inext), 0); }
+            }
+          }
           if (MODE != 0) {
             float res[3];
 #pragma unroll
@@ -1057,6 +1212,8 @@
   io.tile_counters = a.tile_counters;
   io.mask_buf = a.mask_buf; io.mask_cap = a.mask_cap; io.mask_base_host = a.mask_buf ? a.mask_base_host : -1;
   io.mask_base_dev = a.mask_base_dev; io.slots = a.slots; io.sdf_in = a.sdf_in;
+  memset(&io.tail, 0, sizeof(io.tail));
+  io.tail_rows_max = io.tail_far_max = 0;
   DIST_REQUIRE(!io.screen_seg1 || io.seg_approx != nullptr, "tensor-core engine: two-tier precision needs seg_approx");
   DIST_REQUIRE((a.n2_host == 0 && !a.n2_dev) || (a.seg2_offset % 128 == 0 && a.seg2_offset >= a.n_host),
                "tensor-core engine: the second row segment must start at a multiple of 128 behind the first");
@@ -1099,6 +1256,12 @@
   int clusters = num_sms() / 2;
   if (tiles < clusters) clusters = (int)tiles;
   if (clusters < 1) clusters = 1;
+  if (mode == 0 && a.tail && a.tail->on) {
+    DIST_REQUIRE(io.screen_seg1 && a.n2_dev && a.seg2_offset > 0, "tensor-core engine: the march tail needs the two row segments");
+    io.tail = *a.tail;
+    io.tail_rows_max = (int64_t)(a.tail->rows_waves * (float)(clusters * 128));
+    io.tail_far_max = (int64_t)(a.tail->far_waves * (float)(clusters * 128));
+  }
   if (mode == 0) { mlp_tc_kernel<0><<<clusters * 2, NTHREADS, SMEM_BYTES, stream>>>(tmap, tmap_hi, P, io); }
   else if (mode == 1) { mlp_tc_kernel<1><<<clusters * 2, NTHREADS, SMEM_BYTES, stream>>>(tmap, tmap_hi, P, io); }
   else if (mode == 2) { mlp_tc_kernel<2><<<clusters * 2, NTHREADS, SMEM_BYTES, stream>>>(tmap, tmap_hi, P, io); }
diff --git a/dist-renderer_b200/renderer.py b/dist-renderer_b200/renderer.py
--- a/dist-renderer_b200/renderer.py
+++ b/dist-renderer_b200/renderer.py
@@ -44,7 +44,7 @@
         mp.cam_grad_levels = opts["cam_levels"]
         screen = plan.tc.get("screen") if (engine == _abi.ENGINE_TC and plan.tc is not None and ren.screen) else None
         if screen:
-            mp.screen, mp.screen_margin = 1, screen["margin"]
+            mp.screen, mp.screen_margin = 1 | (2 if ren.march_tail else 0), screen["margin"]
             mp.screen_tpred, mp.screen_ext_margin = ren.screen_tpred, ren.screen_ext_margin
         f32 = dict(device=dev, dtype=torch.float32)
         saved = {
@@ -146,7 +146,8 @@
     def __init__(self, decoder, intrinsic, img_hw=None, transform_matrix=None, march_step=50, buffer_size=5,
                  ray_marching_ratio=1.5, use_depth2normal=False, max_sample_dist=0.2, radius=1.0, threshold=5e-5,
                  scale_list=[4, 2, 1], march_step_list=[3, 3, -1], use_gpu=True, is_eval=True, engine=None,
-                 rows=None, screen=None, screen_tpred=0.30, screen_ext_margin=0.04, mask_cache=None, mask_rows_per_ray=9.0):
+                 rows=None, screen=None, screen_tpred=0.30, screen_ext_margin=0.04, mask_cache=None, mask_rows_per_ray=9.0,
+                 march_tail=None):
         self.decoder = decoder
         if use_gpu and torch.cuda.device_count() == 0:
             raise ValueError('No GPU device found.')
@@ -201,6 +202,7 @@
         self.screen_ext_margin = float(os.environ.get("DIST_SCREEN_EXT", screen_ext_margin))
         self.mask_cache = (os.environ.get("DIST_MASK_CACHE", "1") != "0") if mask_cache is None else bool(mask_cache)
         self.mask_rows_per_ray = float(mask_rows_per_ray)
+        self.march_tail = (os.environ.get("DIST_MARCH_TAIL", "1") != "0") if march_tail is None else bool(march_tail)
         self._homo_calib = None
         self._calib_map = None
         self._scr = None
```

After: 8.930 million, median of 6. About the same (-0.5%).
